# gear-genomics/tracy

Hardware: AMD Instinct MI355X
Metric: GCUPS (tracy align: Gotoh affine-gap DP cells per second, whole job) (higher is better)
Workload: dtype int16 (score sweeps) / int32 (tracebacks)

## Files before the change

include/tracy_hip.h:

```cpp
#ifndef TRACY_HIP_H
#define TRACY_HIP_H

#include <stddef.h>
#include <stdint.h>

#ifdef __cplusplus
extern "C" {
#endif

#define TRACYHIP_OK 0
#define TRACYHIP_ERR_ARG (-1)
#define TRACYHIP_ERR_HIP (-2)
#define TRACYHIP_ERR_OOM (-3)
#define TRACYHIP_ERR_RANGE (-4)
#define TRACYHIP_ERR_NODEVICE (-5)

#define TRACYHIP_MEM_HOST 0
#define TRACYHIP_MEM_DEVICE 1

#define TRACYHIP_SEQ_CHAR 0
#define TRACYHIP_SEQ_PROFILE 1

typedef struct tracyhip_ctx tracyhip_ctx;

typedef struct {
  int32_t match;
  int32_t mismatch;
  int32_t go;
  int32_t ge;
  int32_t hfree;
  int32_t vfree;
} tracyhip_params;

typedef struct {
  int32_t kind;
  const void* data;
  const uint64_t* offset;
  const uint32_t* length;
  uint32_t count;
} tracyhip_seqset;

typedef struct {
  uint32_t npairs;
  tracyhip_seqset a1;
  tracyhip_seqset a2;
  const uint32_t* a1_index;
  const uint32_t* a2_index;
} tracyhip_pairs;

int tracyhip_device_count(int* count);
int tracyhip_create(int device, tracyhip_ctx** ctx);
int tracyhip_destroy(tracyhip_ctx* ctx);
int tracyhip_set_stream(tracyhip_ctx* ctx, void* hip_stream);
int tracyhip_set_workspace_limit(tracyhip_ctx* ctx, uint64_t bytes);
int tracyhip_set_lanes(tracyhip_ctx* ctx, uint32_t lanes);
int tracyhip_synchronize(tracyhip_ctx* ctx);
int tracyhip_set_option(tracyhip_ctx* ctx, const char* name, const char* value);
int tracyhip_describe(tracyhip_ctx* ctx, char* buf, size_t cap);
int tracyhip_tune_host_allocator(void);
typedef struct {
  uint32_t traces;
  uint32_t stream_ordered;
  uint32_t host_syncs;
  uint32_t fallback_traces;
  uint32_t pruned;
  uint32_t pruned_uncertified;
  uint32_t prelim_banded;
  uint32_t prelim_repeated;
  uint32_t final_banded;
  uint32_t final_repeated;
  uint32_t allele_pruned[2];
  uint32_t allele_uncertified[2];
  uint32_t allele_banded[3];
  uint32_t allele_repeated[3];
  uint32_t allele_shared_prefix;
  uint32_t cons_fixup_columns;
  uint32_t cons_chunks;
  uint32_t asm_chunks;
  uint32_t asm_steps;
  uint32_t denovo_chunks;
  uint32_t denovo_rounds;
  uint32_t denovo_steps;
  uint32_t var_traces;
  uint32_t var_realigned;
  uint32_t var_truncated;
  uint32_t var_chunks;
  uint32_t sweep_diag_launches;
  uint32_t prefix_diag_launches;
  uint32_t band_list_pairs[2][4];
  uint32_t band_large_launches;
} tracyhip_call_stats;
int tracyhip_last_call_stats(tracyhip_ctx* ctx, tracyhip_call_stats* out);
const char* tracyhip_last_error(void);
const char* tracyhip_version(void);

int tracyhip_gotoh_score(tracyhip_ctx* ctx, const tracyhip_pairs* pairs, const tracyhip_params* prm,
                         int mem, int32_t* scores);
int tracyhip_gotoh_align(tracyhip_ctx* ctx, const tracyhip_pairs* pairs, const tracyhip_params* prm,
                         int mem, int32_t* scores, uint8_t* ops, const uint64_t* ops_offset,
                         uint32_t* ops_len);
int tracyhip_gotoh_banded(tracyhip_ctx* ctx, const tracyhip_pairs* pairs, const tracyhip_params* prm, const int32_t* band_lo,
                          const int32_t* band_hi, int mem, int32_t* scores, uint8_t* ops, const uint64_t* ops_offset, uint32_t* ops_len,
                          uint32_t* ends);
int tracyhip_needle_score(tracyhip_ctx* ctx, const tracyhip_pairs* pairs, const tracyhip_params* prm,
                          int mem, int32_t* scores);
int tracyhip_needle_align(tracyhip_ctx* ctx, const tracyhip_pairs* pairs, const tracyhip_params* prm,
                          int mem, int32_t* scores, uint8_t* ops, const uint64_t* ops_offset,
                          uint32_t* ops_len);
int tracyhip_alignment_rows(tracyhip_ctx* ctx, const tracyhip_pairs* pairs, int mem, const uint8_t* ops,
                            const uint64_t* ops_offset, const uint32_t* ops_len, uint8_t* rows0,
                            uint8_t* rows1);

typedef struct {
  uint32_t ntraces;
  tracyhip_seqset profiles;
  tracyhip_seqset refs;
  const uint32_t* ref_index;
  uint32_t trim_left;
  uint32_t trim_right;
  const uint8_t* oriented;
  uint32_t strand_by_certificate;
} tracyhip_align_job;

typedef struct {
  int32_t* score_fwd;
  int32_t* score_rev;
  uint8_t* forward;
  int32_t* score_prelim;
  uint32_t* slice_begin;
  uint32_t* slice_len;
  uint32_t* ref_pos;
  int32_t* score_final;
  uint8_t* ops;
  const uint64_t* ops_offset;
  uint32_t* ops_len;
} tracyhip_align_result;

int tracyhip_align_traces(tracyhip_ctx* ctx, const tracyhip_align_job* job, const tracyhip_params* prm,
                          int mem, const tracyhip_align_result* out);

typedef struct {
  int32_t indelshift;
  int32_t traceleft;
  uint32_t breakpoint;
  float best_diff;
} tracyhip_breakpoint;

typedef struct {
  uint32_t ntraces;
  const int32_t* signal;
  const uint64_t* signal_offset;
  const uint32_t* nsamples;
  const int32_t* bcpos;
  uint8_t* primary;
  uint8_t* secondary;
  const uint64_t* bc_offset;
  const uint32_t* bc_len;
  const int32_t* peaks;
} tracyhip_basecalls;

typedef struct {
  int32_t trim_left;
  int32_t trim_right;
  int32_t maxindel;
  int32_t madc;
} tracyhip_decomp_params;

typedef struct {
  int32_t kind;
  int32_t best_ins;
  int32_t best_del;
  int32_t best_fr;
  uint32_t dcp_n;
// ... 327 lines not shown
```

tracy_amd/capi.py:

```python
import ctypes as C
import os

import numpy as np

_HERE = os.path.dirname(os.path.abspath(__file__))

OK, ERR_ARG, ERR_HIP, ERR_OOM, ERR_RANGE, ERR_NODEVICE = 0, -1, -2, -3, -4, -5
MEM_HOST, MEM_DEVICE = 0, 1
SEQ_CHAR, SEQ_PROFILE = 0, 1


class TracyHipError(RuntimeError):
    def __init__(self, code, msg):
        super().__init__("tracyhip error %d: %s" % (code, msg))
        self.code = code


class Params(C.Structure):
    _fields_ = [("match", C.c_int32), ("mismatch", C.c_int32), ("go", C.c_int32), ("ge", C.c_int32),
                ("hfree", C.c_int32), ("vfree", C.c_int32)]


class SeqSet(C.Structure):
    _fields_ = [("kind", C.c_int32), ("data", C.c_void_p), ("offset", C.POINTER(C.c_uint64)),
                ("length", C.POINTER(C.c_uint32)), ("count", C.c_uint32)]


class Pairs(C.Structure):
    _fields_ = [("npairs", C.c_uint32), ("a1", SeqSet), ("a2", SeqSet), ("a1_index", C.POINTER(C.c_uint32)),
                ("a2_index", C.POINTER(C.c_uint32))]


class AlignJob(C.Structure):
    _fields_ = [("ntraces", C.c_uint32), ("profiles", SeqSet), ("refs", SeqSet), ("ref_index", C.POINTER(C.c_uint32)),
                ("trim_left", C.c_uint32), ("trim_right", C.c_uint32), ("oriented", C.POINTER(C.c_uint8)),
                ("strand_by_certificate", C.c_uint32)]


class AlignResult(C.Structure):
    _fields_ = [("score_fwd", C.c_void_p), ("score_rev", C.c_void_p), ("forward", C.c_void_p),
                ("score_prelim", C.c_void_p), ("slice_begin", C.c_void_p), ("slice_len", C.c_void_p),
                ("ref_pos", C.c_void_p), ("score_final", C.c_void_p), ("ops", C.c_void_p),
                ("ops_offset", C.POINTER(C.c_uint64)), ("ops_len", C.c_void_p)]


class CallStats(C.Structure):
    _fields_ = [("traces", C.c_uint32), ("stream_ordered", C.c_uint32), ("host_syncs", C.c_uint32), ("fallback_traces", C.c_uint32),
                ("pruned", C.c_uint32), ("pruned_uncertified", C.c_uint32), ("prelim_banded", C.c_uint32), ("prelim_repeated", C.c_uint32),
                ("final_banded", C.c_uint32), ("final_repeated", C.c_uint32), ("allele_pruned", C.c_uint32 * 2),
                ("allele_uncertified", C.c_uint32 * 2), ("allele_banded", C.c_uint32 * 3), ("allele_repeated", C.c_uint32 * 3),
                ("allele_shared_prefix", C.c_uint32), ("cons_fixup_columns", C.c_uint32), ("cons_chunks", C.c_uint32),
                ("asm_chunks", C.c_uint32), ("asm_steps", C.c_uint32),
                ("denovo_chunks", C.c_uint32), ("denovo_rounds", C.c_uint32), ("denovo_steps", C.c_uint32)]


class CallStatsVariants(CallStats):
    _fields_ = [("var_traces", C.c_uint32), ("var_realigned", C.c_uint32), ("var_truncated", C.c_uint32), ("var_chunks", C.c_uint32)]


class CallStatsSweeps(CallStatsVariants):
    _fields_ = [("sweep_diag_launches", C.c_uint32), ("prefix_diag_launches", C.c_uint32)]


class CallStatsBands(CallStatsSweeps):
    _fields_ = [("band_list_pairs", (C.c_uint32 * 4) * 2), ("band_large_launches", C.c_uint32)]


def library_path():
    return os.path.join(_HERE, "lib", "libtracy_hip.so")


_LIB = None


def lib():
    global _LIB
    if _LIB is None:
        p = library_path()
        if not os.path.exists(p):
            raise ImportError("tracy_amd: %s is missing -- run `python tracy_amd/build.py` (hipcc, gfx950). "
                              "There is no CPU fallback." % p)
        _LIB = C.CDLL(p)
        _LIB.tracyhip_last_error.restype = C.c_char_p
        _LIB.tracyhip_version.restype = C.c_char_p
        _LIB.tracyhip_group_context.restype = C.c_void_p
    return _LIB


def _check(rc):
    if rc != OK:
        raise TracyHipError(rc, lib().tracyhip_last_error().decode())


def device_count():
    n = C.c_int(0)
    rc = lib().tracyhip_device_count(C.byref(n))
    return n.value if rc == OK else 0


class PackedSeqs:

    def __init__(self, seqs, kind=None):
        if kind is None:
            kind = SEQ_CHAR if (len(seqs) == 0 or isinstance(seqs[0], (bytes, bytearray))) else SEQ_PROFILE
        self.kind = kind
        self.count = len(seqs)
        self.length = np.zeros(max(self.count, 1), dtype=np.uint32)
        self.offset = np.zeros(max(self.count, 1), dtype=np.uint64)
        pos = 0
        parts = []
        for i, s in enumerate(seqs):
            if kind == SEQ_CHAR:
                a = np.frombuffer(bytes(s), dtype=np.uint8)
                ln = a.size
            else:
                a = np.ascontiguousarray(s, dtype=np.float32)
                assert a.ndim == 2 and a.shape[0] == 6
                ln = a.shape[1]
                a = a.reshape(-1)
            self.length[i] = ln
            self.offset[i] = pos
            pos += a.size
            parts.append(a)
        dt = np.uint8 if kind == SEQ_CHAR else np.float32
        self.data = np.concatenate(parts) if parts and pos else np.zeros(1, dtype=dt)
        self.nelem = pos

    def seqset(self, data_ptr=None):
        s = SeqSet()
        s.kind = self.kind
        s.data = data_ptr if data_ptr is not None else self.data.ctypes.data
        s.offset = self.offset.ctypes.data_as(C.POINTER(C.c_uint64))
        s.length = self.length.ctypes.data_as(C.POINTER(C.c_uint32))
        s.count = self.count
        return s


class Context:
    def __init__(self, device=0):
        self._h = C.c_void_p()
        _check(lib().tracyhip_create(int(device), C.byref(self._h)))

    def close(self):
        if self._h:
            lib().tracyhip_destroy(self._h)
            self._h = C.c_void_p()

    def __del__(self):
        try:
            self.close()
        except Exception:
            pass

    def set_stream(self, stream_ptr):
        _check(lib().tracyhip_set_stream(self._h, C.c_void_p(stream_ptr)))

    def set_workspace_limit(self, nbytes):
        _check(lib().tracyhip_set_workspace_limit(self._h, C.c_uint64(nbytes)))

    def set_lanes(self, n):
        _check(lib().tracyhip_set_lanes(self._h, C.c_uint32(n)))

    def synchronize(self):
        _check(lib().tracyhip_synchronize(self._h))

    def set_option(self, name, value):
        _check(lib().tracyhip_set_option(self._h, str(name).encode(), str(int(value) if isinstance(value, bool) else value).encode()))

    def describe(self):
        n = lib().tracyhip_describe(self._h, None, C.c_size_t(0))
        buf = C.create_string_buffer(n)
        lib().tracyhip_describe(self._h, buf, C.c_size_t(n))
        return dict(line.split("=", 1) for line in buf.value.decode().splitlines())

    def last_call_stats(self):
        st = CallStatsBands()
        _check(lib().tracyhip_last_call_stats(self._h, C.byref(st)))
        out = {}
        for name, ty in CallStats._fields_ + CallStatsVariants._fields_ + CallStatsSweeps._fields_ + CallStatsBands._fields_:
            v = getattr(st, name)
            if name == "band_list_pairs":
                out[name] = [list(row) for row in v]
                continue
            out[name] = list(v) if hasattr(v, "__len__") else int(v)
        return out

    @staticmethod
    def _pairs(a1, a2, idx1=None, idx2=None):
        p1 = a1 if isinstance(a1, PackedSeqs) else PackedSeqs(a1)
        p2 = a2 if isinstance(a2, PackedSeqs) else PackedSeqs(a2)
        pr = Pairs()
        keep = [p1, p2]
        if idx1 is not None:
            idx1 = np.ascontiguousarray(idx1, dtype=np.uint32)
            idx2 = np.ascontiguousarray(idx2, dtype=np.uint32)
            pr.npairs = len(idx1)
            pr.a1_index = idx1.ctypes.data_as(C.POINTER(C.c_uint32))
            pr.a2_index = idx2.ctypes.data_as(C.POINTER(C.c_uint32))
            keep += [idx1, idx2]
        else:
            assert p1.count == p2.count
            pr.npairs = p1.count
        pr.a1 = p1.seqset()
        pr.a2 = p2.seqset()
        return pr, keep, p1, p2

    def _pair_lengths(self, pr, p1, p2, idx1, idx2):
        if idx1 is None:
            return p1.length[:pr.npairs].astype(np.uint64), p2.length[:pr.npairs].astype(np.uint64)
        return p1.length[np.asarray(idx1)].astype(np.uint64), p2.length[np.asarray(idx2)].astype(np.uint64)

    def score(self, a1, a2, params, needle=False, idx1=None, idx2=None):
        pr, keep, p1, p2 = self._pairs(a1, a2, idx1, idx2)
        prm = Params(*params)
        out = np.zeros(max(pr.npairs, 1), dtype=np.int32)
        fn = lib().tracyhip_needle_score if needle else lib().tracyhip_gotoh_score
        _check(fn(self._h, C.byref(pr), C.byref(prm), MEM_HOST, out.ctypes.data_as(C.POINTER(C.c_int32))))
        return out[:pr.npairs]

    def align(self, a1, a2, params, needle=False, idx1=None, idx2=None, rows=False):
        pr, keep, p1, p2 = self._pairs(a1, a2, idx1, idx2)
        prm = Params(*params)
        n = pr.npairs
        l1, l2 = self._pair_lengths(pr, p1, p2, idx1, idx2)
        cap = (l1 + l2).astype(np.uint64)
        off = np.zeros(max(n, 1), dtype=np.uint64)
        if n:
            off[1:n] = np.cumsum(cap)[:-1]
        total = int(cap.sum()) if n else 0
        ops = np.zeros(max(total, 1), dtype=np.uint8)
        olen = np.zeros(max(n, 1), dtype=np.uint32)
        scores = np.zeros(max(n, 1), dtype=np.int32)
        fn = lib().tracyhip_needle_align if needle else lib().tracyhip_gotoh_align
        _check(fn(self._h, C.byref(pr), C.byref(prm), MEM_HOST, scores.ctypes.data_as(C.POINTER(C.c_int32)),
                  ops.ctypes.data_as(C.POINTER(C.c_uint8)), off.ctypes.data_as(C.POINTER(C.c_uint64)),
                  olen.ctypes.data_as(C.POINTER(C.c_uint32))))
        btr = [ops[int(off[i]):int(off[i]) + int(olen[i])].tobytes() for i in range(n)]
        if not rows:
            return scores[:n], btr
        r0 = np.zeros(max(total, 1), dtype=np.uint8)
        r1 = np.zeros(max(total, 1), dtype=np.uint8)
        _check(lib().tracyhip_alignment_rows(self._h, C.byref(pr), MEM_HOST, ops.ctypes.data_as(C.POINTER(C.c_uint8)),
                                             off.ctypes.data_as(C.POINTER(C.c_uint64)),
                                             olen.ctypes.data_as(C.POINTER(C.c_uint32)),
                                             r0.ctypes.data_as(C.POINTER(C.c_uint8)),
                                             r1.ctypes.data_as(C.POINTER(C.c_uint8))))
        rws = [(r0[int(off[i]):int(off[i]) + int(olen[i])].tobytes(), r1[int(off[i]):int(off[i]) + int(olen[i])].tobytes())
               for i in range(n)]
        return scores[:n], btr, rws


def _align_banded(self, a1, a2, params, band_lo, band_hi, origin=False):
    pr, keep, p1, p2 = self._pairs(a1, a2, None, None)
    prm = Params(*params)
    n = pr.npairs
    l1, l2 = self._pair_lengths(pr, p1, p2, None, None)
    cap = (l1 + l2).astype(np.uint64)
    off = np.zeros(max(n, 1), dtype=np.uint64)
    if n:
        off[1:n] = np.cumsum(cap)[:-1]
    ops = np.zeros(max(int(cap.sum()) if n else 0, 1), dtype=np.uint8)
    olen = np.zeros(max(n, 1), dtype=np.uint32)
# ... 1096 lines not shown
```

tracy_amd/csrc/band16.hip:

```cpp
#include <hip/hip_runtime.h>

#include "band16.h"
#include "band16_launch.h"
#include "front.h"

namespace tracyhip {

struct DeviceWave16 {
  __device__ __forceinline__ uint32_t lane() const { return threadIdx.x; }
  __device__ __forceinline__ int32_t rot16(int32_t x) const { return __builtin_amdgcn_update_dpp(0, x, 0x121, 0xf, 0xf, false); }
  __device__ __forceinline__ int32_t rot(int32_t x, std::integral_constant<int, 16>) const { return rot16(x); }
  __device__ __forceinline__ int32_t rot(int32_t x, std::integral_constant<int, 4>) const { return __builtin_amdgcn_update_dpp(0, x, 0x93, 0xf, 0xf, false); }
  __device__ __forceinline__ uint64_t ballot(bool p) const { return __ballot(p); }
  __device__ __forceinline__ uint32_t bcast(uint32_t x, uint32_t src_lane) const { return (uint32_t)__shfl((int)x, (int)src_lane, 64); }
  __device__ __forceinline__ void sync() const { __syncthreads(); }
  __device__ __forceinline__ void sync_global() const {
    __builtin_amdgcn_fence(__ATOMIC_RELEASE, "workgroup");
    __builtin_amdgcn_fence(__ATOMIC_ACQUIRE, "workgroup");
  }
  __device__ __forceinline__ char* lds() const {
    extern __shared__ __attribute__((aligned(16))) char tracy_smem16[];
    return tracy_smem16;
  }
};

template <int K, int KIND>
__global__ __launch_bounds__(64) void band16_kernel(Band16Args a) {
  DeviceWave16 w;
  band16_body<DeviceWave16, K, KIND>(w, a, blockIdx.x);
}
template <int KIND>
__global__ __launch_bounds__(64) void band16_multi_kernel(Band16Args a12, uint32_t w12, Band16Args a8, uint32_t w8, Band16Args a4) {
  DeviceWave16 w;
  if (blockIdx.x < w12) band16_body<DeviceWave16, 12, KIND>(w, a12, blockIdx.x);
  else if (blockIdx.x < w12 + w8) band16_body<DeviceWave16, 8, KIND>(w, a8, blockIdx.x - w12);
  else band16_body<DeviceWave16, 4, KIND>(w, a4, blockIdx.x - w12 - w8);
}

template <int KIND>
__global__ __launch_bounds__(64) void band16_multi_counted_kernel(Band16Args a12, Band16Args a8, Band16Args a4, Band16Args aq) {
  DeviceWave16 w;
  const uint32_t w12 = (*a12.count + 3u) / 4u, w8 = (*a8.count + 3u) / 4u, w4 = (*a4.count + 3u) / 4u, wq = (*aq.count + 15u) / 16u;
  if (blockIdx.x < w12) band16_body<DeviceWave16, 12, KIND>(w, a12, blockIdx.x);
  else if (blockIdx.x < w12 + w8) band16_body<DeviceWave16, 8, KIND>(w, a8, blockIdx.x - w12);
  else if (blockIdx.x < w12 + w8 + w4) band16_body<DeviceWave16, 4, KIND>(w, a4, blockIdx.x - w12 - w8);
  else if (blockIdx.x < w12 + w8 + w4 + wq) band16_body<DeviceWave16, 4, KIND, false, 4>(w, aq, blockIdx.x - w12 - w8 - w4);
}

template <int KIND>
__global__ __launch_bounds__(64) void band16_multi3_counted_kernel(Band16Args a8, Band16Args a4, Band16Args aq) {
  DeviceWave16 w;
  const uint32_t w8 = (*a8.count + 3u) / 4u, w4 = (*a4.count + 3u) / 4u, wq = (*aq.count + 15u) / 16u;
  if (blockIdx.x < w8) band16_body<DeviceWave16, 8, KIND>(w, a8, blockIdx.x);
  else if (blockIdx.x < w8 + w4) band16_body<DeviceWave16, 4, KIND>(w, a4, blockIdx.x - w8);
  else if (blockIdx.x < w8 + w4 + wq) band16_body<DeviceWave16, 4, KIND, false, 4>(w, aq, blockIdx.x - w8 - w4);
}

template <int K>
__global__ __launch_bounds__(64) void band16_cont_kernel(Band16Args a) {
  DeviceWave16 w;
  band16_body<DeviceWave16, K, 1, true>(w, a, blockIdx.x);
}

template <int K>
__global__ __launch_bounds__(64) void band16_cont16_kernel(Band16Args a) {
  DeviceWave16 w;
  band16_cont16_body<DeviceWave16, K>(w, a, blockIdx.x);
}

__global__ __launch_bounds__(64) void band16_cont16_quad_kernel(Band16Args a) {
  DeviceWave16 w;
  band16_cont16_body<DeviceWave16, 4, 4>(w, a, blockIdx.x);
}

__global__ __launch_bounds__(64) void front_place_kernel(const FrontDesc* __restrict__ desc, const uint32_t* __restrict__ row, int32_t goe, int32_t halfw,
                                                         PairDesc* __restrict__ pairs, FrontOut* __restrict__ fo, const FrontOut* __restrict__ prev,
                                                         const uint32_t* __restrict__ index, const uint32_t* __restrict__ count) {
  DeviceWave16 w;
  uint32_t u = blockIdx.x;
  if (index) {
    if (u >= *count) return;
    u = index[u];
  }
  FrontDesc f = desc[u];
  if (prev && prev[u].ok) f.flags |= PAIR_SKIP;
  const FrontOut* known = (prev && !(f.flags & PAIR_SKIP) && prev[u].cstar != 0u) ? prev + u : nullptr;
  front_place_body(w, f, row, goe, halfw, pairs + u, fo + u, known);
}
__global__ __launch_bounds__(64) void front_certify_kernel(const FrontDesc* __restrict__ desc, const uint32_t* __restrict__ row, int32_t go, int32_t ge,
                                                           int32_t halfw, const int32_t* __restrict__ scores, const uint32_t* __restrict__ ends,
                                                           FrontOut* __restrict__ fo, const FrontOut* __restrict__ prev,
                                                           const uint32_t* __restrict__ index, const uint32_t* __restrict__ count) {
  DeviceWave16 w;
  uint32_t u = blockIdx.x;
  if (index) {
    if (u >= *count) return;
    u = index[u];
  }
  const FrontDesc f = desc[u];
  if (prev && prev[u].ok) return;
  front_certify_body(w, f, row, go, ge, halfw, scores[f.out], ends[2 * f.out + 1], fo + u);
}

__global__ __launch_bounds__(256) void b16_table_kernel(const B16TableDesc* __restrict__ desc, const void* __restrict__ a1, int strings,
                                                        int32_t match, int32_t mismatch, int32_t qlimit, int shift, int16_t* __restrict__ out,
                                                        int32_t* __restrict__ err) {
  const B16TableDesc d = desc[blockIdx.x];
  bool overflow = false;
  int32_t qabs = 0;
  for (uint32_t r = threadIdx.x; r < d.stride; r += blockDim.x) {
    const bool real = r < d.m;
    int32_t q[kB16Codes] = {0, 0, 0, 0, 0, 0};
    if (real) {
      b16_table_row(a1, strings != 0, d.a1_off, d.a1_stride, r, match, mismatch, q);
      if (!strings)
        for (uint32_t b = 0; b < 5; ++b) qabs = imax(qabs, q[b] < 0 ? -q[b] : q[b]);
    }
#pragma unroll
    for (uint32_t b = 0; b < kB16Codes; ++b) {
      const int32_t v = (int32_t)((uint32_t)q[b] << shift);
      overflow |= v > 32767 || v < -32768 || q[b] > 32767 || q[b] < -32768;
      out[d.out_off + (uint64_t)b * d.stride + r] = (int16_t)v;
    }
  }
  if (overflow) flag_error(err, 1);
  if (!strings && qabs > qlimit) flag_max(err, 1, qabs);
}

hipError_t launch_b16_tables(const B16TableDesc* d_desc, uint32_t nseq, const void* a1, bool strings, int32_t match, int32_t mismatch,
                             int32_t qlimit, int shift, int16_t* out, int32_t* err, hipStream_t s) {
  if (nseq == 0) return hipSuccess;
  hipLaunchKernelGGL(b16_table_kernel, dim3(nseq), dim3(256), 0, s, d_desc, a1, strings ? 1 : 0, match, mismatch, qlimit, shift, out, err);
  return hipGetLastError();
}

hipError_t launch_band16(int K, int kind, const Band16Args& a, hipStream_t s) {
  if (a.npairs == 0) return hipSuccess;
  const dim3 grid((a.npairs + 3u) / 4u);
  const uint32_t lds = 4u * a.code_cap + b16_table_bytes(K);
#define TRACY_B16(KK)                                                                                     \
  case KK:                                                                                                \
    if (kind == 0) hipLaunchKernelGGL((band16_kernel<KK, 0>), grid, dim3(64), lds, s, a);                 \
    else hipLaunchKernelGGL((band16_kernel<KK, 1>), grid, dim3(64), lds, s, a);                           \
    break;
  switch (K) {
    TRACY_B16(4) TRACY_B16(8) TRACY_B16(12)
    default: return hipErrorInvalidValue;
  }
#undef TRACY_B16
  return hipGetLastError();
}

hipError_t launch_band16_multi(int kind, const Band16Args& a12, const Band16Args& a8, const Band16Args& a4, hipStream_t s) {
  const uint32_t w12 = (a12.npairs + 3u) / 4u, w8 = (a8.npairs + 3u) / 4u, w4 = (a4.npairs + 3u) / 4u;
  if (w12 + w8 + w4 == 0) return hipSuccess;
  const uint32_t lds = 4u * a12.code_cap + b16_table_bytes(12);
  if (kind == 0) hipLaunchKernelGGL((band16_multi_kernel<0>), dim3(w12 + w8 + w4), dim3(64), lds, s, a12, w12, a8, w8, a4);
  else hipLaunchKernelGGL((band16_multi_kernel<1>), dim3(w12 + w8 + w4), dim3(64), lds, s, a12, w12, a8, w8, a4);
  return hipGetLastError();
}

hipError_t B16Fork::create() {
  hipError_t e;
  int least = 0, greatest = 0;
  if (hipDeviceGetStreamPriorityRange(&least, &greatest) != hipSuccess) { (void)hipGetLastError(); least = greatest = 0; }
  const bool flat = getenv("TRACYHIP_NO_STREAM_PRIORITY") != nullptr;
  for (int i = 0; i < kSide; ++i) {
    const int prio = (!flat && i == 3) ? least : 0;
    (void)greatest;
    if ((e = hipStreamCreateWithPriority(&side[i], hipStreamNonBlocking, prio)) != hipSuccess) return e;
// ... 3 lines not shown
    if ((e = hipEventCreateWithFlags(&r, hipEventDisableTiming)) != hipSuccess) return e;
  return hipEventCreateWithFlags(&forked, hipEventDisableTiming);
}
void B16Fork::destroy() {
  for (int i = 0; i < kSide; ++i) {
    if (side[i]) (void)hipStreamDestroy(side[i]);
    if (joined[i]) (void)hipEventDestroy(joined[i]);
    side[i] = nullptr; joined[i] = nullptr;
  }
  for (auto& r : ready) { if (r) (void)hipEventDestroy(r); r = nullptr; }
  if (forked) (void)hipEventDestroy(forked);
  forked = nullptr;
}

hipError_t launch_band16_counted(int kind, const Band16Args& a12, const Band16Args& a8, const Band16Args& a4, const Band16Args& aq, hipStream_t s,
                                 const B16Fork* fork, uint32_t multi_max, bool* large) {
  if (large) *large = false;
  uint32_t most = a12.npairs;
  for (uint32_t x : {a8.npairs, a4.npairs, aq.npairs}) most = x > most ? x : most;
  if (most == 0) return hipSuccess;
  hipError_t e;
  if (most <= multi_max) {
    const uint32_t lds16 = 4u * a12.code_cap + b16_table_bytes(12), ldsq = aq.npairs ? b16_quad_lds(aq.code_cap) : 0u;
    const uint32_t lds = lds16 > ldsq ? lds16 : ldsq;
    const dim3 grid((most + 3u) / 4u + 4u);
    if (kind == 0) hipLaunchKernelGGL((band16_multi_counted_kernel<0>), grid, dim3(64), lds, s, a12, a8, a4, aq);
    else hipLaunchKernelGGL((band16_multi_counted_kernel<1>), grid, dim3(64), lds, s, a12, a8, a4, aq);
    return hipGetLastError();
  }
  if (large) *large = true;
  const uint32_t lds16 = 4u * a8.code_cap + b16_table_bytes(8), ldsq = aq.npairs ? b16_quad_lds(aq.code_cap) : 0u;
  const uint32_t lds = lds16 > ldsq ? lds16 : ldsq;
  const dim3 grid((most + 3u) / 4u + 3u);
  if (fork) {
    if ((e = hipEventRecord(fork->forked, s)) != hipSuccess) return e;
    if ((e = hipStreamWaitEvent(fork->side[2], fork->forked, 0)) != hipSuccess) return e;
  }
  if (kind == 0) hipLaunchKernelGGL((band16_multi3_counted_kernel<0>), grid, dim3(64), lds, s, a8, a4, aq);
  else hipLaunchKernelGGL((band16_multi3_counted_kernel<1>), grid, dim3(64), lds, s, a8, a4, aq);
  if ((e = hipGetLastError()) != hipSuccess) return e;
  if ((e = launch_band16(12, kind, a12, fork ? fork->side[2] : s)) != hipSuccess) return e;
  if (fork) {
    if ((e = hipEventRecord(fork->joined[2], fork->side[2])) != hipSuccess) return e;
    if ((e = hipStreamWaitEvent(s, fork->joined[2], 0)) != hipSuccess) return e;
  }
  return hipSuccess;
}

hipError_t launch_band16_cont_quad(const Band16Args& a, hipStream_t s) {
  if (a.npairs == 0) return hipSuccess;
  hipLaunchKernelGGL(band16_cont16_quad_kernel, dim3((a.npairs + 15u) / 16u), dim3(64), b16_cont_quad_lds(a.code_cap), s, a);
  return hipGetLastError();
}

hipError_t launch_band16_cont(int K, const Band16Args& a, hipStream_t s, bool narrow) {
  if (a.npairs == 0) return hipSuccess;
  const dim3 grid((a.npairs + 3u) / 4u);
  const uint32_t lds = narrow ? b16_cont16_lds(K, a.code_cap) : 4u * a.code_cap + b16_table_bytes(K) + 4u * 2u * kB16RowCap * 4u;
  if (narrow) {
    switch (K) {
      case 12: hipLaunchKernelGGL((band16_cont16_kernel<12>), grid, dim3(64), lds, s, a); break;
      case 8: hipLaunchKernelGGL((band16_cont16_kernel<8>), grid, dim3(64), lds, s, a); break;
      case 4: hipLaunchKernelGGL((band16_cont16_kernel<4>), grid, dim3(64), lds, s, a); break;
      default: return hipErrorInvalidValue;
    }
    return hipGetLastError();
  }
  switch (K) {
    case 12: hipLaunchKernelGGL((band16_cont_kernel<12>), grid, dim3(64), lds, s, a); break;
    case 8: hipLaunchKernelGGL((band16_cont_kernel<8>), grid, dim3(64), lds, s, a); break;
    case 4: hipLaunchKernelGGL((band16_cont_kernel<4>), grid, dim3(64), lds, s, a); break;
    default: return hipErrorInvalidValue;
  }
  return hipGetLastError();
}

hipError_t launch_front_place(const FrontDesc* d_desc, uint32_t n, const uint32_t* row, int32_t goe, int32_t halfw, PairDesc* d_pairs, FrontOut* d_fo,
                              hipStream_t s, const FrontOut* d_prev, const uint32_t* d_index, const uint32_t* d_count) {
  if (n == 0) return hipSuccess;
  hipLaunchKernelGGL(front_place_kernel, dim3(n), dim3(64), 0, s, d_desc, row, goe, halfw, d_pairs, d_fo, d_prev, d_index, d_count);
  return hipGetLastError();
}

hipError_t launch_front_certify(const FrontDesc* d_desc, uint32_t n, const uint32_t* row, int32_t go, int32_t ge, int32_t halfw, const int32_t* d_scores,
                                const uint32_t* d_ends, FrontOut* d_fo, hipStream_t s, const FrontOut* d_prev, const uint32_t* d_index,
                                const uint32_t* d_count) {
  if (n == 0) return hipSuccess;
  hipLaunchKernelGGL(front_certify_kernel, dim3(n), dim3(64), 0, s, d_desc, row, go, ge, halfw, d_scores, d_ends, d_fo, d_prev, d_index, d_count);
  return hipGetLastError();
}

}
```

tracy_amd/csrc/band16_launch.h:

```cpp
#ifndef TRACY_AMD_BAND16_LAUNCH_H
#define TRACY_AMD_BAND16_LAUNCH_H

#include <hip/hip_runtime.h>

#include "band16.h"

namespace tracyhip {

struct B16TableDesc {
  uint64_t a1_off;
  uint64_t out_off;
  uint32_t a1_stride;
  uint32_t m;
  uint32_t stride;
  uint32_t pad;
};

hipError_t launch_b16_tables(const B16TableDesc* d_desc, uint32_t nseq, const void* a1, bool strings, int32_t match, int32_t mismatch,
                             int32_t qlimit, int shift, int16_t* out, int32_t* err, hipStream_t s);
hipError_t launch_band16(int K, int kind, const Band16Args& a, hipStream_t s);
hipError_t launch_band16_multi(int kind, const Band16Args& a12, const Band16Args& a8, const Band16Args& a4, hipStream_t s);
struct B16Fork {
  static constexpr int kSide = 4;
  hipStream_t side[kSide] = {nullptr, nullptr, nullptr, nullptr};
  hipEvent_t forked = nullptr, joined[kSide] = {nullptr, nullptr, nullptr, nullptr};
  hipEvent_t ready[2] = {nullptr, nullptr};
  hipError_t create();
  void destroy();
};
#ifndef TRACY_B16_MULTI_MAX
#define TRACY_B16_MULTI_MAX 49152u
#endif
hipError_t launch_band16_counted(int kind, const Band16Args& a12, const Band16Args& a8, const Band16Args& a4, const Band16Args& aq, hipStream_t s,
                                 const B16Fork* fork = nullptr, uint32_t multi_max = TRACY_B16_MULTI_MAX, bool* large = nullptr);
hipError_t launch_band16_cont(int K, const Band16Args& a, hipStream_t s, bool narrow = false);
hipError_t launch_band16_cont_quad(const Band16Args& a, hipStream_t s);
struct FrontDesc;
struct FrontOut;
hipError_t launch_front_place(const FrontDesc* d_desc, uint32_t n, const uint32_t* row, int32_t goe, int32_t halfw, PairDesc* d_pairs, FrontOut* d_fo,
                              hipStream_t s, const FrontOut* d_prev = nullptr, const uint32_t* d_index = nullptr, const uint32_t* d_count = nullptr);
hipError_t launch_front_certify(const FrontDesc* d_desc, uint32_t n, const uint32_t* row, int32_t go, int32_t ge, int32_t halfw, const int32_t* d_scores,
                                const uint32_t* d_ends, FrontOut* d_fo, hipStream_t s, const FrontOut* d_prev = nullptr, const uint32_t* d_index = nullptr,
                                const uint32_t* d_count = nullptr);

}
#endif
```

tracy_amd/csrc/capi.hip:

```cpp
#include <hip/hip_runtime.h>
#include <atomic>
#include <sched.h>
#include <malloc.h>
#include <map>
#include <chrono>

#include <thread>

#include <algorithm>
#include <cctype>
#include <cstdarg>
#include <cstddef>
#include <cstdio>
#include <cstdlib>
#include <cstring>
#include <string>
#include <memory>
#include <vector>

#include "../../include/tracy_hip.h"
#include "capi_internal.h"
#include "launch.h"
#include "stream_plan.h"
#include "sweep_range.h"
// ... 128 lines not shown
      {
        std::unique_lock<std::mutex> lk(m);
        cv.wait(lk, [&] { return gen != seen; });
        seen = gen;
        j = job;
      }
      slices(*j);
      {
        std::lock_guard<std::mutex> lk(m);
        if (--pending == 0) done_cv.notify_one();
      }
    }
  }
  static uint32_t share() {
    uint32_t want = kHostThreads;
    if (const char* e = getenv("TRACYHIP_HOST_THREADS")) { const int v = atoi(e); if (v >= 1) want = (uint32_t)v; }
    else {
      cpu_set_t set;
      CPU_ZERO(&set);
      if (sched_getaffinity(0, sizeof(set), &set) == 0) { const int c = CPU_COUNT(&set); if (c >= 1) want = (uint32_t)c; }
      if (FILE* f = fopen("/sys/fs/cgroup/cpu.max", "r")) {
        char quota[32] = {0};
        unsigned long period = 0;
        if (fscanf(f, "%31s %lu", quota, &period) == 2 && period > 0 && strcmp(quota, "max") != 0) {
          const unsigned long q = strtoul(quota, nullptr, 10) / period;
          if (q >= 1 && q < want) want = (uint32_t)q;
        }
        fclose(f);
      }
    }
    return want > kHostThreads ? kHostThreads : want;
  }
  bool run(const std::function<void(uint32_t)>& f) {
    std::unique_lock<std::mutex> u(use, std::try_to_lock);
    if (!u.owns_lock()) return false;
    if (!started) {
      const uint32_t want = share();
      nworkers = want - 1;
      for (uint32_t t = 0; t < nworkers; ++t) std::thread([this] { worker(); }).detach();
      started = true;
    }
    {
      std::lock_guard<std::mutex> lk(m);
      job = &f;
      next.store(0);
      pending = nworkers;
      ++gen;
    }
    if (nworkers) cv.notify_all();
    slices(f);
    std::unique_lock<std::mutex> lk(m);
    done_cv.wait(lk, [&] { return pending == 0; });
    return true;
  }
};
}
uint32_t host_pool_threads() {
  static const uint32_t n = HostPool::share();
  return n;
}
bool host_pool_run(const std::function<void(uint32_t)>& job) {
  static HostPool* pool = new HostPool;
  return pool->run(job);
}

HostScope::HostScope(const char* l) : label(l), t0(host_profile().on ? now_ns() : 0) {}
HostScope::~HostScope() {
  HostProfile& p = host_profile();
  if (!p.on) return;
  const double ms = (double)(now_ns() - t0) * 1e-6;
  std::lock_guard<std::mutex> lk(p.m);
  auto& e = p.acc[label];
  e.first += ms;
  e.second += 1;
}

namespace {
struct KnobField { const char* name; bool CtxKnobs::*flag; };
const KnobField kKnobFlags[] = {
    {"no_stream", &CtxKnobs::no_stream}, {"no_narrow", &CtxKnobs::no_narrow}, {"no_compact", &CtxKnobs::no_compact},
    {"no_screen", &CtxKnobs::no_screen}, {"no_band", &CtxKnobs::no_band}, {"no_band16", &CtxKnobs::no_band16},
    {"no_front", &CtxKnobs::no_front}, {"no_prefix", &CtxKnobs::no_prefix}, {"no_vote", &CtxKnobs::no_vote},
    {"no_origin", &CtxKnobs::no_origin}, {"no_subwindow", &CtxKnobs::no_subwindow}, {"no_prelim_origin", &CtxKnobs::no_prelim_origin},
    {"no_cq", &CtxKnobs::no_cq}, {"no_fused_walk", &CtxKnobs::no_fused_walk}, {"no_cont16", &CtxKnobs::no_cont16}, {"no_decomp_wave", &CtxKnobs::no_decomp_wave}, {"no_af_split", &CtxKnobs::no_af_split}, {"no_front_lists", &CtxKnobs::no_front_lists}, {"no_origin_band", &CtxKnobs::no_origin_band}, {"no_quads", &CtxKnobs::no_quads}, {"no_fork", &CtxKnobs::no_fork}, {"no_early_tail", &CtxKnobs::no_early_tail}, {"sweeps_alone", &CtxKnobs::sweeps_alone}, {"no_sweep_diag", &CtxKnobs::no_sweep_diag}, {"verbose", &CtxKnobs::verbose}};
bool same_name(const char* a, const char* b) {
  for (; *a && *b; ++a, ++b)
    if (std::tolower((unsigned char)*a) != std::tolower((unsigned char)*b)) return false;
  return *a == *b;
}
}
bool knobs_set(CtxKnobs& k, const char* name, const char* value) {
  if (!name || !value) return false;
  if (same_name(name, "band_w")) {
    char* end = nullptr;
    const long v = strtol(value, &end, 10);
    if (end == value) return false;
    k.band_w = v < 0 ? -1 : (int32_t)std::min<long>(4096, v);
    return true;
  }
  if (same_name(name, "quad_tier_min")) {
    const long v = atol(value);
    if (v < 0) return false;
    k.quad_tier_min = (uint32_t)std::min<long>(v, 0x7fffffffl);
    return true;
  }
  if (same_name(name, "front_list_min")) {
    const long v = atol(value);
    if (v < 0) return false;
    k.front_list_min = (uint32_t)std::min<long>(v, 0x7fffffffl);
    return true;
  }
  if (same_name(name, "b16_multi_max")) {
    char* end = nullptr;
    const long v = strtol(value, &end, 10);
    if (end == value || *end || v < 0 || v > 0x7fffffffl) return false;
    k.b16_multi_max = (uint32_t)v;
    return true;
  }
  if (same_name(name, "seed_vote_cap")) {
    const long v = atol(value);
    if (v < 1 || v > 2048) return false;
    k.seed_vote_cap = (uint32_t)v;
    return true;
  }
  if (same_name(name, "sweep_diag_period")) {
    const long v = atol(value);
    if (v != 0 && (v < 64 || v > 32768 || v % 4 != 0)) return false;
    k.sweep_diag_period = (uint32_t)v;
    return true;
  }
  if (same_name(name, "ckpt_b")) {
    const long v = atol(value);
    if (v < 32 || v > 1024) return false;
    k.ckpt_b = (uint32_t)v;
    return true;
  }
  for (const KnobField& f : kKnobFlags)
    if (same_name(name, f.name)) {
      k.*(f.flag) = !(value[0] == '0' && value[1] == 0);
      return true;
    }
  return false;
}
void knobs_from_env(CtxKnobs& k) {
  for (const KnobField& f : kKnobFlags) {
    std::string env = "TRACYHIP_";
    for (const char* c = f.name; *c; ++c) env.push_back((char)std::toupper((unsigned char)*c));
    if (getenv(env.c_str())) k.*(f.flag) = true;
  }
  if (getenv("TRACYHIP_HOST_TIMERS")) k.verbose = true;
  if (const char* e = getenv("TRACYHIP_BAND_W")) knobs_set(k, "band_w", e);
  if (const char* e = getenv("TRACYHIP_CKPT_B")) knobs_set(k, "ckpt_b", e);
  if (const char* e = getenv("TRACYHIP_QUAD_TIER_MIN")) knobs_set(k, "quad_tier_min", e);
  if (const char* e = getenv("TRACYHIP_FRONT_LIST_MIN")) knobs_set(k, "front_list_min", e);
  if (const char* e = getenv("TRACYHIP_B16_MULTI_MAX")) knobs_set(k, "b16_multi_max", e);
  if (const char* e = getenv("TRACYHIP_SEED_VOTE_CAP")) knobs_set(k, "seed_vote_cap", e);
  if (const char* e = getenv("TRACYHIP_SWEEP_DIAG_PERIOD")) knobs_set(k, "sweep_diag_period", e);
}
std::string knobs_describe(const CtxKnobs& k) {
  std::string s;
  for (const KnobField& f : kKnobFlags) { s += f.name; s += k.*(f.flag) ? "=1\n" : "=0\n"; }
  s += "band_w=" + std::to_string(k.band_w) + "\n";
  s += "ckpt_b=" + std::to_string(k.ckpt_b) + "\n";
  s += "quad_tier_min=" + std::to_string(k.quad_tier_min) + "\n";
  s += "front_list_min=" + std::to_string(k.front_list_min) + "\n";
  s += "b16_multi_max=" + std::to_string(k.b16_multi_max) + "\n";
  s += "seed_vote_cap=" + std::to_string(k.seed_vote_cap) + "\n";
// ... 1422 lines not shown
```

tracy_amd/csrc/capi_internal.h:

```cpp
#ifndef TRACY_AMD_CAPI_INTERNAL_H
#define TRACY_AMD_CAPI_INTERNAL_H

#include <hip/hip_runtime.h>

#include <atomic>
#include <condition_variable>
#include <deque>
#include <functional>
#include <mutex>
#include <string>
#include <thread>
#include <utility>
#include <vector>

#include "../../include/tracy_hip.h"
#include "assemble_wave.h"
#include "dp_kernels.h"
#include "band16_launch.h"
#include "front.h"

namespace tracyhip {

struct DevBuf {
  void* p = nullptr;
// ... 91 lines not shown
  AB_OFF,
  AB_LEN,
  AB_W0,
  AB_W1,
  AB_SPAN,
  AB_PROF,
  AB_PCLASS,
  AB_STEP,
  AB_PAY,
  DN_PROF = AB_TR,
  DN_SEQS = AB_SEQS,
  DN_CLASS = AB_CLASS,
  DN_COLCLASS = AB_PCLASS,
  DN_TABLE = AB_SC2,
  DN_OPS = AB_OPS,
  DN_OFF = AB_OFF,
  DN_LEN = AB_LEN,
  DN_ROWS = AB_W0,
  DN_SPAN = AB_SPAN,
  DN_STEP = AB_STEP,
  DN_PAY = AB_PAY,
  DN_CNT,
  VB_DESC,
  VB_EVENTS,
  VB_LEN,
  VB_PAIRS,
  VB_RCDESC,
  VB_SEQ,
  VB_OPS,
  VB_OPS_OFF,
  VB_OPS_LEN,
  VB_IN_PRIMARY,
  VB_IN_SECDECOMP,
  VB_IN_REFS,
  VB_IN_OPS0,
  VB_IN_OPS1,
  VB_OUT_REC,
  VB_OUT_TEXT,
  VB_OUT_N,
  VB_PACK_OFF,
  VB_PACK_REC,
  VB_PACK_TEXT,
  DB_COUNT
};
static_assert(DN_CNT + 1 == VB_DESC && VB_PACK_TEXT + 1 == DB_COUNT && DN_PAY < DB_COUNT,
              "an alias does not advance the count: every slot of its own comes after the aliases");
enum CtxPin : int {
  PB_DESC,
  PB_OFF,
  PB_TMP,
  PB_RES,
  PB_PRE,
  PB_B16DESC0,
  PB_COUNT = PB_B16DESC0 + 4
};

int set_error(int code, const char* fmt, ...);
#define HIP_TRY(expr)                                                                               \
  do {                                                                                              \
    hipError_t _e = (expr);                                                                         \
    if (_e != hipSuccess)                                                                           \
      return set_error(_e == hipErrorOutOfMemory ? TRACYHIP_ERR_OOM : TRACYHIP_ERR_HIP, "%s failed: %s (%s:%d)", \
                       #expr, hipGetErrorString(_e), __FILE__, __LINE__);                           \
  } while (0)

struct CtxKnobs {
  bool no_stream = false;
  bool no_narrow = false;
  bool no_compact = false;
  bool no_screen = false;
  bool no_band = false;
  bool no_band16 = false;
  bool no_front = false;
  bool no_prefix = false;
  bool no_vote = false;
  bool no_origin = false;
  bool no_subwindow = false;
  bool no_prelim_origin = false;
  bool no_cq = false;
  bool no_fused_walk = false;
  bool no_quads = false;
  bool no_fork = false;
  bool no_early_tail = false;
  bool sweeps_alone = false;
  bool no_sweep_diag = false;
  bool no_origin_band = false;
  bool no_front_lists = false;
  bool no_af_split = false;
  bool no_decomp_wave = false;
  bool no_cont16 = false;
  bool verbose = false;
  int32_t band_w = -1;
  uint32_t ckpt_b = 256;
  uint32_t sweep_diag_period = 0;
  uint32_t b16_multi_max = TRACY_B16_MULTI_MAX;
  uint32_t front_list_min = 1024;
  uint32_t seed_vote_cap = 2048;
  uint32_t quad_tier_min = 32768;
};
void knobs_from_env(CtxKnobs& k);
bool knobs_set(CtxKnobs& k, const char* name, const char* value);
std::string knobs_describe(const CtxKnobs& k);

constexpr size_t kCodePad = 128;
int choose_k(uint32_t m, int mode, bool needle = false);
uint64_t seqset_extent(const tracyhip_seqset& s);

struct DpProblem {
  int mode = MODE_CHAR;
  bool a1_profile = false, a2_profile = false;
  const void* d_a1 = nullptr;
  const void* d_a2 = nullptr;
  const void* d_a2_chars = nullptr;
  const uint8_t* d_special = nullptr;
  int cq_codes = 6;
  const uint8_t* d_colclass = nullptr;
  std::vector<PairDesc> desc;
  std::vector<int> k;
};

}

struct tracyhip_ctx {
  int device = 0;
  hipStream_t stream = nullptr;
  hipStream_t own_stream = nullptr;
  uint64_t ws_limit = 0;
  tracyhip::DevBuf dev[tracyhip::DB_COUNT];
  tracyhip::PinBuf pin[tracyhip::PB_COUNT];
  std::vector<tracyhip::PairDesc> cache_desc;
  std::vector<int> cache_k;
  std::vector<tracyhip::PairDesc> cache_full, cache_pre, cache_b16;
  std::vector<tracyhip::FrontDesc> cache_fd;
  std::vector<int> cache_fullk, cache_b16k;
  tracyhip::B16Fork b16_fork;
  bool b16_fork_ok = false;
  bool cons_gq_ready = false;
  hipError_t ensure_codes(size_t bytes, hipStream_t st) {
    tracyhip::DevBuf &d_codes = dev[tracyhip::DB_CODES], &d_special = dev[tracyhip::DB_SPECIAL];
    hipError_t e = d_codes.ensure(bytes + 2 * tracyhip::kCodePad);
    if (e != hipSuccess) return e;
    if ((e = hipMemsetAsync(d_codes.p, 0, tracyhip::kCodePad, st)) != hipSuccess) return e;
    if ((e = hipMemsetAsync(static_cast<uint8_t*>(d_codes.p) + tracyhip::kCodePad + bytes, 0, tracyhip::kCodePad, st)) != hipSuccess) return e;
    if ((e = d_special.ensure((bytes >> 8) + 2)) != hipSuccess) return e;
    return hipMemsetAsync(d_special.p, 0, (bytes >> 8) + 2, st);
  }
  uint8_t* special_blocks() const { return static_cast<uint8_t*>(dev[tracyhip::DB_SPECIAL].p); }
  uint8_t* codes() const { return static_cast<uint8_t*>(dev[tracyhip::DB_CODES].p) + tracyhip::kCodePad; }
  bool aftab_ready = false;
  uint64_t ws_cache_budget = 0, ws_cache_held = 0;
  uint32_t ws_cache_share = 0;
  bool declut_ready = false;
  uint32_t b16_round = 0;
  struct Pending { int which; hipEvent_t e0, e1; uint64_t cells, bytes; };
  std::vector<tracyhip_ctx*> lanes;
  uint32_t mem_share = 1;
  bool timing = false;
  tracyhip::CtxKnobs knobs;
  tracyhip_call_stats stats = {};
  std::vector<Pending> pending;
  std::vector<hipEvent_t> free_events;
  tracyhip_kernel_timing acc[TRACYHIP_TIMER_COUNT] = {};
  struct AsyncState {
    std::mutex m;
    std::condition_variable cv;
    std::deque<std::function<int()>> q;
// ... 167 lines not shown
```

tracy_amd/csrc/dp_kernels.h:

```cpp
#ifndef TRACY_AMD_DP_KERNELS_H
#define TRACY_AMD_DP_KERNELS_H

#include "dp_lane.h"

#if defined(__HIP_DEVICE_COMPILE__)
#define TRACY_KEEP_BRANCH() asm volatile("" ::: "memory")
#else
#define TRACY_KEEP_BRANCH() ((void)0)
#endif

namespace tracyhip {

enum : int { MODE_CHAR = 0, MODE_QP = 1, MODE_PROF = 2, MODE_CQ = 3 };
TR_HD constexpr bool qp_like(int mode) { return mode == MODE_QP || mode == MODE_CQ; }
TR_HD uint32_t cq_code(uint8_t c) { return c == 'A' ? 0u : c == 'C' ? 1u : c == 'G' ? 2u : c == 'T' ? 3u : c == 'N' ? 4u : 5u; }
TR_HD bool cq_row_char(uint8_t c) { return c == 'A' || c == 'C' || c == 'G' || c == 'T' || c == 'N'; }
enum : uint32_t {
  PAIR_A2_REVCOMP = 1u,
  PAIR_ROW4_ZERO = 2u,
  PAIR_BANDED = 4u,
  PAIR_KEEP_ROW = 8u,
  PAIR_SKIP = 16u,
};

// ... 502 lines not shown
#pragma unroll
          for (int k = 0; k < 5; ++k) nb[k] = a2p[(uint64_t)k * d.a2_stride + ci];
        }
        bool screen_on = screen_pair;
        uint32_t nfail = 0;
        const uint8_t* cls = screen_on ? a.colcode + d.a2_off : nullptr;
        uint32_t ncls = kColClassOther;
        if (screen_on) {
          sub.screen_setup();
          ncls = cls[col_at(1 - (int32_t)L)];
        }
        for (uint32_t t = 1; t <= t_end; ++t) {
#pragma unroll
          for (int k = 0; k < 5; ++k) sub.b[k] = nb[k];
          const uint32_t ccls = ncls;
          const uint32_t ci = col_at((int32_t)t - (int32_t)L + 1);
#pragma unroll
          for (int k = 0; k < 5; ++k) nb[k] = a2p[(uint64_t)k * d.a2_stride + ci];
          if (screen_on) {
            ncls = cls[ci];
            int32_t bad = sub.screen();
            if (ccls < kColClassOther) {
              const int16_t* tp = qp_tab + qp6_index<K>(ccls, 0u, L);
#pragma unroll
              for (int i = 0; i < K; ++i) sub.sv[i] = (int32_t)((uint32_t)(int32_t)tp[i * 64] << SH);
              bad = 0;
            }
            if (w.ballot(bad < 0) != 0) {
              sub.prepare();
              if (++nfail > 64u && 2u * nfail > t) screen_on = false;
            }
          } else {
            sub.prepare();
          }
          do_step(t, sub);
        }
      };
      auto sweep4 = [&]() {
        SubProf<K, 4> s4;
#pragma unroll
        for (int i = 0; i < K; ++i)
#pragma unroll
          for (int k = 0; k < 5; ++k) s4.a[i][k] = sub_p.a[i][k];
        s4.fmatch = fmatch; s4.fmis = fmis; s4.shift = SH;
        sweep(s4);
      };
      if constexpr (NT == 4) sweep4();
      else if constexpr (NT == 5) sweep(sub_p);
      else { if (skip4) sweep4(); else sweep(sub_p); }
    }
    (void)T;

    if (BOTTOM) {
      if (a.scores && L == lanes_used - 1) a.scores[d.out] = NARROW ? sext16(bot_h - goe) : bot_h;
    } else if (last_pass && a.scores) {
      const uint32_t g = m - 1 - base;
      if (L == g / K) {
        int32_t v = 0;
#pragma unroll
        for (int i = 0; i < K; ++i)
          if ((uint32_t)i == g % K) v = TRACE ? (ts.Hc[i] >> SH) : ((NARROW || A16) ? sext16(ss.Hl[i]) : ss.Hl[i]);
        a.scores[d.out] = v;
      }
    }
    if (!last_pass) w.sync_global();
  }
}

template <bool G>
struct SweepGuard { static constexpr bool value = G; };

template <int K>
struct QpStrip {
  uint32_t v[K];
  TR_HD int32_t lo16(int i) const { return (int32_t)v[i]; }
};
TR_HD constexpr uint32_t lds_bytes_sweep16(int K, bool compact) { return (compact ? 4u : 6u) * 256u * (uint32_t)((K + 1) / 2); }
TR_HD constexpr uint32_t lds_bytes_prefix(int K, bool compact) { return lds_bytes_sweep16(K, compact); }
template <int NC>
TR_HD constexpr uint32_t qp16_row_byte(uint32_t row) { return (row >> 1) * ((uint32_t)NC * 256u) + (row & 1u) * 128u; }
template <int NC>
TR_HD uint32_t qp16_byte(uint32_t code, uint32_t row, uint32_t lanecol) { return qp16_row_byte<NC>(row) + code * 256u + 2u * lanecol; }
template <class W>
TR_HD bool reference_is_plain(W& w, const DpArgs& a, const PairDesc& d) {
  if (!a.special_blocks) return false;
  if (d.n == 0) return true;
  const uint64_t first = d.a2_off >> 8, last = (d.a2_off + d.n - 1) >> 8;
  uint32_t seen = 0;
  for (uint64_t b = first + w.lane(); b <= last; b += 64) seen |= a.special_blocks[b];
  return w.ballot(seen != 0) == 0;
}
template <int K, int NC>
TR_HD void qp_fetch6(const char* tab, uint32_t addr, QpStrip<K>& q) {
#if defined(__HIP_DEVICE_COMPILE__)
#pragma unroll
  for (int i = 0; i < K; ++i) asm volatile("ds_read_u16 %0, %1 offset:%2" : "=v"(q.v[i]) : "v"(addr), "n"(qp16_row_byte<NC>((uint32_t)i)));
#else
  for (int i = 0; i < K; ++i) {
    uint16_t x;
    __builtin_memcpy(&x, tab + addr + qp16_row_byte<NC>((uint32_t)i), 2);
    q.v[i] = x;
  }
#endif
}
template <int K>
TR_HD void qp_wait6(QpStrip<K>& q) {
#if defined(__HIP_DEVICE_COMPILE__)
  constexpr int newer = K < 15 ? K : 15;
#define TR_TIE4(o) "+v"(q.v[o]), "+v"(q.v[o + 1]), "+v"(q.v[o + 2]), "+v"(q.v[o + 3])
  if constexpr (K == 15) asm volatile("s_waitcnt lgkmcnt(%15)" : TR_TIE4(0), TR_TIE4(4), TR_TIE4(8), "+v"(q.v[12]), "+v"(q.v[13]), "+v"(q.v[14]) : "n"(newer));
  else if constexpr (K == 16) asm volatile("s_waitcnt lgkmcnt(%16)" : TR_TIE4(0), TR_TIE4(4), TR_TIE4(8), TR_TIE4(12) : "n"(newer));
  else if constexpr (K == 12) asm volatile("s_waitcnt lgkmcnt(%12)" : TR_TIE4(0), TR_TIE4(4), TR_TIE4(8) : "n"(newer));
  else if constexpr (K == 8) asm volatile("s_waitcnt lgkmcnt(%8)" : TR_TIE4(0), TR_TIE4(4) : "n"(newer));
  else if constexpr (K == 4) asm volatile("s_waitcnt lgkmcnt(%4)" : TR_TIE4(0) : "n"(newer));
  else asm volatile("s_waitcnt lgkmcnt(0)" ::: "memory");
#undef TR_TIE4
#endif
}

TR_HD int32_t lastrow_h(const int32_t* lr, uint32_t c, bool narrow) { return narrow ? sext16(lr[c]) : lr[2 * c]; }
TR_HD int32_t lastrow_e(const int32_t* lr, uint32_t c, bool narrow, int32_t goe) { return narrow ? (lr[c] >> 16) + goe : lr[2 * c + 1]; }

template <class W, int K, bool CKPT, bool COMPACT, bool STRINGS, bool DIAG>
TR_HD void gotoh_narrow_qp_body(W& w, const DpArgs& a, uint32_t pair_idx) {
  const PairDesc d = a.pairs[pair_idx];
  if (d.flags & PAIR_SKIP) return;
  if (reference_is_plain(w, a, d) != COMPACT) return;
  const uint32_t L = w.lane();
  const uint32_t m = d.m, n = d.n;
  const int32_t go = a.go, ge = a.ge, goe = go + ge;
  if (m == 0 || n == 0) {
    if (L == 0 && a.scores) a.scores[d.out] = (m == 0) ? 0 : edge_value(false, go, ge, (int32_t)m);
    return;
  }
  const float* a1p = static_cast<const float*>(a.a1) + (STRINGS ? 0 : d.a1_off);
  const uint8_t* a1c = static_cast<const uint8_t*>(a.a1) + (STRINGS ? d.a1_off : 0);
  const uint8_t* a2c = static_cast<const uint8_t*>(a.a2) + d.a2_off;
  constexpr int NC = COMPACT ? 4 : 6;
  int16_t* qp_tab = reinterpret_cast<int16_t*>(w.lds());
  const float fmatch = (float)a.match, fmis = (float)a.mismatch;
  const uint32_t lanes_used = (m + K - 1) / K;
  const uint32_t pad = lanes_used * K - m;
  const uint32_t t_end = n + lanes_used - 1;
  const bool rcflag = (d.flags & PAIR_A2_REVCOMP) != 0;
  const bool lastlane = L == lanes_used - 1;

  int32_t Hl[K], El[K];
#pragma unroll
  for (int i = 0; i < K; ++i) {
    const uint32_t r = L * K + i + 1 - pad;
    if constexpr (DIAG) {
      const int32_t rr = (int32_t)(L * K + i + 1) - (int32_t)pad;
      if (rr <= 0) { Hl[i] = rr * -ge; El[i] = -goe + (rr - 1) * -ge; }
      else { Hl[i] = go; El[i] = kNegInf16 + (rr - 1) * -ge; }
    } else if (L * K + i < pad) { Hl[i] = 0; El[i] = -goe; }
    else { Hl[i] = edge_value(false, go, ge, (int32_t)r); El[i] = kNegInf16; }
  }
  int32_t gev = ge, goev = DIAG ? go : goe;
  int32_t hext_last = lastlane ? (DIAG ? -ge : 0) : (DIAG ? 0 : ge);
  int32_t delta_last = lastlane ? -goe : 0;
#if defined(__HIP_DEVICE_COMPILE__)
  asm volatile("" : "+v"(gev), "+v"(goev), "+v"(hext_last), "+v"(delta_last));
#endif

  const uint32_t Lc = ((L & 31u) << 1) | (L >> 5);
  {
    bool overflow = false;
    int32_t qabs = 0;
#pragma unroll 1
    for (int i = 0; i < K; ++i) {
      const uint32_t r = L * K + i + 1 - pad;
      const bool real = r - 1 < m;
      float pr[5] = {0.0f, 0.0f, 0.0f, 0.0f, 0.0f};
// ... 1217 lines not shown
```

tracy_amd/csrc/dp_kernels.hip:

```cpp
#include <hip/hip_runtime.h>

#include <cstdlib>

#include "dp_kernels.h"
#include "launch.h"

namespace tracyhip {

static uint32_t lds_pad() {
  static int v = -1;
  if (v < 0) { const char* e = getenv("TRACYHIP_LDS_PAD"); v = e ? atoi(e) : 0; }
  return (uint32_t)v;
}

struct DeviceWave {
  __device__ __forceinline__ uint32_t lane() const { return threadIdx.x; }
  __device__ __forceinline__ int32_t shift_up(int32_t x) const {
    return __builtin_amdgcn_update_dpp(0, x, 0x138, 0xf, 0xf, true);
  }
  __device__ __forceinline__ int32_t shift_up_row(int32_t x) const {
    return __builtin_amdgcn_update_dpp(0, x, 0x111, 0xf, 0xf, true);
  }
  __device__ __forceinline__ int32_t shift_up_or(int32_t x, int32_t first) const {
    return __builtin_amdgcn_update_dpp(first, x, 0x138, 0xf, 0xf, false);
// ... 424 lines not shown
  if (mode == MODE_CHAR) return launch_band_m<MODE_CHAR>(K, a, wa, npairs, s);
  if (mode == MODE_QP) return launch_band_m<MODE_QP>(K, a, wa, npairs, s);
  return hipErrorInvalidValue;
}

hipError_t launch_gotoh_origin(int K, int table, int codes, const DpArgs& a, uint32_t npairs, hipStream_t s) {
  if (npairs == 0) return hipSuccess;
  if (table == 2) {
#define TRACY_ORIGIN_QP(KK)                                                                                                            \
  case KK:                                                                                                                              \
    if (a.special_blocks) hipLaunchKernelGGL((gotoh_origin_kernel<KK, 2, 4>), dim3(npairs), dim3(64), 4u * 64u * KK * 2u + lds_pad(), s, a); \
    hipLaunchKernelGGL((gotoh_origin_kernel<KK, 2, 6>), dim3(npairs), dim3(64), lds_bytes(MODE_QP, KK), s, a);                              \
    break;
    switch (K) {
      TRACY_ORIGIN_QP(4) TRACY_ORIGIN_QP(8) TRACY_ORIGIN_QP(12) TRACY_ORIGIN_QP(15) TRACY_ORIGIN_QP(16)
      default: return hipErrorInvalidValue;
    }
#undef TRACY_ORIGIN_QP
    return hipGetLastError();
  }
  if (table) {
#define TRACY_ORIGIN_CASE(KK)                                                                                                          \
  case KK:                                                                                                                              \
    if (codes <= 4) hipLaunchKernelGGL((gotoh_origin_kernel<KK, 1, 4>), dim3(npairs), dim3(64), 4u * 64u * KK * 2u + lds_pad(), s, a);      \
    else if (codes == 5) hipLaunchKernelGGL((gotoh_origin_kernel<KK, 1, 5>), dim3(npairs), dim3(64), 5u * 64u * KK * 2u + lds_pad(), s, a); \
    else hipLaunchKernelGGL((gotoh_origin_kernel<KK, 1, 6>), dim3(npairs), dim3(64), lds_bytes(MODE_CQ, KK), s, a);                          \
    break;
    switch (K) {
      TRACY_ORIGIN_CASE(4) TRACY_ORIGIN_CASE(8) TRACY_ORIGIN_CASE(12) TRACY_ORIGIN_CASE(15) TRACY_ORIGIN_CASE(16)
      default: return hipErrorInvalidValue;
    }
#undef TRACY_ORIGIN_CASE
    return hipGetLastError();
  }
  switch (K) {
    case 4: hipLaunchKernelGGL((gotoh_origin_kernel<4>), dim3(npairs), dim3(64), 0, s, a); break;
    case 8: hipLaunchKernelGGL((gotoh_origin_kernel<8>), dim3(npairs), dim3(64), 0, s, a); break;
    case 12: hipLaunchKernelGGL((gotoh_origin_kernel<12>), dim3(npairs), dim3(64), 0, s, a); break;
    case 15: hipLaunchKernelGGL((gotoh_origin_kernel<15>), dim3(npairs), dim3(64), 0, s, a); break;
    case 16: hipLaunchKernelGGL((gotoh_origin_kernel<16>), dim3(npairs), dim3(64), 0, s, a); break;
    default: return hipErrorInvalidValue;
  }
  return hipGetLastError();
}

static constexpr uint32_t lds_combo(int K, bool compact) {
  const uint32_t pre = lds_bytes_prefix(K, compact), sw = lds_bytes_sweep16(K, compact);
  return pre > sw ? pre : sw;
}
hipError_t launch_gotoh_ckpt_prefix(int K, const DpArgs& full, uint32_t nfull, const DpArgs& pre, uint32_t npre, hipStream_t s) {
  if (nfull + npre == 0) return hipSuccess;
  constexpr int GL = kPrefixLanes;
  const dim3 grid(nfull + (npre + 64 / GL - 1) / (64 / GL));
#define TRACY_COMBO_CASE(KK)                                                                                            \
  case KK:                                                                                                              \
    if constexpr (KK == 15 || KK == 16) {                                                                               \
      if (combo_uses_diag<KK>(full, nfull, pre, npre)) {                                                                \
        if (full.special_blocks)                                                                                        \
          hipLaunchKernelGGL((gotoh_ckpt_prefix_kernel<KK, GL, true, KK, true>), grid, dim3(64), lds_combo(KK, true), s, full, nfull, pre, npre); \
        hipLaunchKernelGGL((gotoh_ckpt_prefix_kernel<KK, GL, false, KK, true>), grid, dim3(64), lds_combo(KK, false), s, full, nfull, pre, npre); \
        break;                                                                                                          \
      }                                                                                                                 \
    }                                                                                                                   \
    if (full.special_blocks) {                                                                                          \
      hipLaunchKernelGGL((gotoh_ckpt_prefix_kernel<KK, GL, true>), grid, dim3(64), lds_combo(KK, true), s, full, nfull, pre, npre); \
      hipLaunchKernelGGL((gotoh_ckpt_prefix_kernel<KK, GL, false>), grid, dim3(64), lds_combo(KK, false), s, full, nfull, pre, npre); \
    } else {                                                                                                            \
      hipLaunchKernelGGL((gotoh_ckpt_prefix_kernel<KK, GL, false>), grid, dim3(64), lds_combo(KK, false), s, full, nfull, pre, npre); \
    }                                                                                                                   \
    break;
  switch (K) {
    TRACY_COMBO_CASE(4) TRACY_COMBO_CASE(8) TRACY_COMBO_CASE(12) TRACY_COMBO_CASE(15) TRACY_COMBO_CASE(16)
    default: return hipErrorInvalidValue;
  }
#undef TRACY_COMBO_CASE
  return hipGetLastError();
}

static uint32_t front_prefix_tall_min() {
  static const uint32_t v = [] { const char* e = getenv("TRACYHIP_PREFIX_TALL_MIN"); return e ? (uint32_t)strtoul(e, nullptr, 10) : 40000u; }();
  return v;
}
template <int GL, int KP>
static hipError_t launch_gotoh_ckpt_front_t(int K, const DpArgs& full, uint32_t nfull, const DpArgs& pre, uint32_t npre, hipStream_t s) {
  static_assert(GL * KP == (int)kFrontRows, "the rows above the kept one");
  const dim3 grid(nfull + (npre + 64 / GL - 1) / (64 / GL));
  auto lds = [](int KK, bool compact) {
    const uint32_t pre_b = lds_bytes_prefix(KP, compact), sw = lds_bytes_sweep16(KK, compact);
    return (pre_b > sw ? pre_b : sw) + lds_pad();
  };
#define TRACY_FRONT_CASE(KK)                                                                                            \
  case KK:                                                                                                              \
    if constexpr (KK == 15 || KK == 16) {                                                                               \
      if (combo_uses_diag<KK>(full, nfull, pre, npre)) {                                                                \
        if (full.special_blocks)                                                                                        \
          hipLaunchKernelGGL((gotoh_ckpt_prefix_kernel<KK, GL, true, KP, true>), grid, dim3(64), lds(KK, true), s, full, nfull, pre, npre); \
        hipLaunchKernelGGL((gotoh_ckpt_prefix_kernel<KK, GL, false, KP, true>), grid, dim3(64), lds(KK, false), s, full, nfull, pre, npre); \
        break;                                                                                                          \
      }                                                                                                                 \
    }                                                                                                                   \
    if (full.special_blocks) {                                                                                          \
       \
       \
      hipLaunchKernelGGL((gotoh_ckpt_prefix_kernel<KK, GL, true, KP>), grid, dim3(64), lds(KK, true), s, full, nfull, pre, npre); \
      hipLaunchKernelGGL((gotoh_ckpt_prefix_kernel<KK, GL, false, KP>), grid, dim3(64), lds(KK, false), s, full, nfull, pre, npre); \
    } else {                                                                                                            \
      hipLaunchKernelGGL((gotoh_ckpt_prefix_kernel<KK, GL, false, KP>), grid, dim3(64), lds(KK, false), s, full, nfull, pre, npre); \
    }                                                                                                                   \
    break;
  switch (K) {
    TRACY_FRONT_CASE(4) TRACY_FRONT_CASE(8) TRACY_FRONT_CASE(12) TRACY_FRONT_CASE(15) TRACY_FRONT_CASE(16)
    default: return hipErrorInvalidValue;
  }
#undef TRACY_FRONT_CASE
  return hipGetLastError();
}
hipError_t launch_gotoh_ckpt_front(int K, const DpArgs& full, uint32_t nfull, const DpArgs& pre, uint32_t npre, hipStream_t s) {
  if (nfull + npre == 0) return hipSuccess;
  if (nfull == 0 && npre >= front_prefix_tall_min()) return launch_gotoh_ckpt_front_t<(int)kFrontRows / 16, 16>(K, full, nfull, pre, npre, s);
  return launch_gotoh_ckpt_front_t<kFrontPrefixLanes, kFrontPrefixK>(K, full, nfull, pre, npre, s);
}

hipError_t launch_gotoh_prefix(int K, const DpArgs& a, uint32_t npairs, hipStream_t s) {
  if (npairs == 0) return hipSuccess;
  constexpr int GL = kPrefixLanes;
  const dim3 grid((npairs + 64 / GL - 1) / (64 / GL));
#define TRACY_PREFIX_CASE(KK) \
  case KK:                                                                                                                      \
    hipLaunchKernelGGL((gotoh_prefix_kernel<KK, GL, false>), grid, dim3(64), lds_bytes_prefix(KK, false), s, a, npairs);                        \
    if (a.special_blocks) hipLaunchKernelGGL((gotoh_prefix_kernel<KK, GL, true>), grid, dim3(64), lds_bytes_prefix(KK, true), s, a, npairs); \
    break;
  switch (K) {
    TRACY_PREFIX_CASE(4) TRACY_PREFIX_CASE(8) TRACY_PREFIX_CASE(12) TRACY_PREFIX_CASE(15) TRACY_PREFIX_CASE(16)
    default: return hipErrorInvalidValue;
  }
#undef TRACY_PREFIX_CASE
  return hipGetLastError();
}
template <int GL, int KP>
static hipError_t launch_gotoh_front_prefix_cq_t(const DpArgs& a, uint32_t npairs, hipStream_t s) {
  const dim3 grid((npairs + 64 / GL - 1) / (64 / GL));
  hipLaunchKernelGGL((gotoh_prefix_kernel<KP, GL, false, true>), grid, dim3(64), lds_bytes_prefix(KP, false), s, a, npairs);
  if (a.special_blocks) hipLaunchKernelGGL((gotoh_prefix_kernel<KP, GL, true, true>), grid, dim3(64), lds_bytes_prefix(KP, true), s, a, npairs);
  return hipGetLastError();
}
hipError_t launch_gotoh_front_prefix_cq(const DpArgs& a, uint32_t npairs, hipStream_t s) {
  if (npairs == 0) return hipSuccess;
  if (npairs >= front_prefix_tall_min()) return launch_gotoh_front_prefix_cq_t<(int)kFrontRows / 16, 16>(a, npairs, s);
  return launch_gotoh_front_prefix_cq_t<kFrontPrefixLanes, kFrontPrefixK>(a, npairs, s);
}
hipError_t launch_gotoh_walk(const WalkArgs& a, hipStream_t s) {
  if (a.npairs == 0) return hipSuccess;
  hipLaunchKernelGGL(gotoh_walk_kernel, dim3(a.npairs), dim3(64), 0, s, a);
  return hipGetLastError();
}
hipError_t launch_needle_walk(const WalkArgs& a, const uint32_t* bits32, hipStream_t s) {
  if (a.npairs == 0) return hipSuccess;
  hipLaunchKernelGGL(needle_walk_kernel, dim3((a.npairs + 63) / 64), dim3(64), 0, s, a, bits32);
  return hipGetLastError();
}
hipError_t launch_alignment_rows(const RowsArgs& a, hipStream_t s) {
  if (a.npairs == 0) return hipSuccess;
  hipLaunchKernelGGL(alignment_rows_kernel, dim3(a.npairs), dim3(64), 0, s, a);
  return hipGetLastError();
}

}
```

tracy_amd/csrc/front.h:

```cpp
#ifndef TRACY_AMD_FRONT_H
#define TRACY_AMD_FRONT_H

#include "band16.h"

namespace tracyhip {

constexpr int kFrontK = 12;
constexpr int32_t kFrontHalfW = 90;

struct FrontDesc {
  uint64_t row_off;
  uint64_t a2_off;
  uint64_t tab_off;
  uint32_t tab_stride;
  uint32_t m_rest;
  uint32_t n;
  uint32_t flags;
  uint32_t out;
  uint32_t R;
  int32_t rest;
  uint32_t tight;
};
struct FrontOut {
  int32_t vmax;
  uint32_t cstar;
  uint32_t shift;
  uint32_t ok;
};

TR_HD int32_t front_v(uint32_t x, int32_t goe) {
  const int32_t h = sext16((int32_t)x) - goe, f = (int32_t)x >> 16;
  return h > f ? h : f;
}

template <class W>
TR_HD void front_place_body(W& w, const FrontDesc& f, const uint32_t* row, int32_t goe, int32_t halfw, PairDesc* pair, FrontOut* fo,
                            const FrontOut* known = nullptr) {
  const uint32_t L = w.lane();
  if (f.flags & PAIR_SKIP) {
    if (L == 0) {
      PairDesc d{};
      d.flags = PAIR_SKIP;
      d.out = f.out;
      *pair = d;
      *fo = FrontOut{0, 0u, 0u, 0u};
    }
    return;
  }
  int32_t vmax = INT32_MIN;
  uint32_t cstar = 0;
  if (known) {
    vmax = known->vmax;
    cstar = known->cstar;
  } else {
    const uint32_t* r = row + f.row_off;
    int32_t best = INT32_MIN;
    uint32_t bc = 0;
    constexpr uint32_t kRounds = 8;
    for (uint32_t c0 = 1u; c0 <= f.n; c0 += 64u * kRounds) {
      uint32_t x[kRounds];
#pragma unroll
      for (uint32_t u = 0; u < kRounds; ++u) {
        const uint32_t c = c0 + 64u * u + L;
        x[u] = r[c <= f.n ? c : f.n];
      }
#pragma unroll
      for (uint32_t u = 0; u < kRounds; ++u) {
        const uint32_t c = c0 + 64u * u + L;
        const int32_t v = front_v(x[u], goe);
        const bool take = c <= f.n && v > best;
        best = take ? v : best;
        bc = take ? c : bc;
      }
    }
    for (uint32_t l = 0; l < 64u; ++l) {
      const int32_t v = (int32_t)w.bcast((uint32_t)best, l);
      const uint32_t c = w.bcast(bc, l);
      if (c != 0 && (v > vmax || (v == vmax && c < cstar))) { vmax = v; cstar = c; }
    }
  }
  if (L != 0) return;
  const int32_t dlo = (int32_t)cstar - halfw, dhi = (int32_t)cstar + halfw;
  const uint32_t a = dlo > 1 ? (uint32_t)(dlo - 1) : 0u;
  uint32_t nsub = f.n - a;
  const uint64_t reach = (uint64_t)f.m_rest + (uint64_t)(dhi - (int32_t)a) + 1ull;
  if ((uint64_t)nsub > reach) nsub = (uint32_t)reach;
  PairDesc d{};
  d.a1_off = f.tab_off;
  d.a1_stride = f.tab_stride;
  d.m = f.m_rest;
  d.n = nsub;
  d.a2_stride = nsub;
  d.a2_off = (f.flags & PAIR_A2_REVCOMP) ? f.a2_off + (uint64_t)(f.n - a - nsub) : f.a2_off + a;
  d.out = f.out;
  d.flags = f.flags & PAIR_A2_REVCOMP;
  d.ckpt_off = band_pack(dlo - (int32_t)a, dhi - (int32_t)a);
  d.lastrow_off = f.row_off + a;
  d.bits_off = f.R;
  *pair = d;
  fo->vmax = vmax;
  fo->cstar = cstar;
  fo->shift = a;
  fo->ok = 0;
}

template <class W>
TR_HD void front_certify_body(W& w, const FrontDesc& f, const uint32_t* row, int32_t go, int32_t ge, int32_t halfw, int32_t score, uint32_t c_end,
                              FrontOut* fo) {
  const uint32_t L = w.lane();
  if (f.flags & PAIR_SKIP) return;
  const uint32_t* r = row + f.row_off;
  const int32_t goe = go + ge;
  const int64_t age = -(int64_t)ge;
  const int64_t dlo = (int64_t)fo->cstar - halfw, dhi = (int64_t)fo->cstar + halfw;
  const bool two = f.tight != 0u && age >= 2;
  const int64_t rest1 = (int64_t)f.rest - ((int64_t)f.tight - 1);
  const int64_t q = age - 1;
  bool bad = false, bad1 = false;
  constexpr uint32_t kRounds = 8;
  for (uint32_t c0 = 0; c0 <= f.n; c0 += 64u * kRounds) {
    uint32_t x[kRounds];
#pragma unroll
    for (uint32_t u = 0; u < kRounds; ++u) {
      const uint32_t c = c0 + 64u * u + L;
      x[u] = f.n ? r[c == 0 ? 1u : c <= f.n ? c : f.n] : 0u;
    }
#pragma unroll
    for (uint32_t u = 0; u < kRounds; ++u) {
      const uint32_t c = c0 + 64u * u + L;
      const int64_t v = c == 0 ? (int64_t)edge_value(false, go, ge, (int32_t)f.R) : (int64_t)front_v(x[u], goe);
      const int64_t cc = (int64_t)c;
      const bool live = c <= f.n;
      const bool inside = cc >= dlo && cc <= dhi;
      const int64_t margin = inside ? (cc - dlo < dhi - cc ? cc - dlo : dhi - cc) : -1;
      bad = bad || (live && v + (int64_t)f.rest - age * (margin + 1) >= (int64_t)score);
      if (two) {
        const int64_t ph = age * (dhi - cc + 1), pv = q * (cc - dlo + 1);
        const int64_t pen = inside ? (ph < pv ? ph : pv) : 0;
        bad1 = bad1 || (live && v + rest1 - pen >= (int64_t)score);
      }
    }
  }
  const bool any = w.ballot(bad) != 0;
  const bool any1 = !two || w.ballot(bad1) != 0;
  if (L == 0) fo->ok = ((!any || !any1) && c_end != 0) ? 1u : 0u;
}

}
#endif
```

tracy_amd/csrc/launch.h:

```cpp
#ifndef TRACY_AMD_LAUNCH_H
#define TRACY_AMD_LAUNCH_H

#include <hip/hip_runtime.h>

#include "dp_kernels.h"

namespace tracyhip {

struct RowsArgs {
  const PairDesc* pairs;
  const void* a1;
  const void* a2;
  int32_t a1_profile, a2_profile;
  int32_t a2_revcomp_flag;
  int32_t a2_onehot;
  const uint8_t* ops;
  const uint64_t* ops_off;
  const uint32_t* ops_len;
  uint8_t* rows0;
  uint8_t* rows1;
  uint32_t npairs;
  const int32_t* row0_gaps_only;
  uint32_t row0_gaps_only_stride;
};

hipError_t launch_gotoh(int mode, int K, bool trace, bool narrow, const DpArgs& a, uint32_t npairs, hipStream_t s, bool rawtab = false);
hipError_t launch_gotoh_front_prefix_cq(const DpArgs& a, uint32_t npairs, hipStream_t s);
hipError_t launch_gotoh_prof(int K, bool trace, bool row4_zero, bool arith16, const DpArgs& a, uint32_t npairs, hipStream_t s);
hipError_t launch_gotoh_ckpt(int mode, int K, bool narrow, const DpArgs& a, uint32_t npairs, hipStream_t s);
hipError_t launch_band_trace(int mode, int K, const DpArgs& a, const WalkArgs& wa, uint32_t npairs, hipStream_t s);
hipError_t launch_gotoh_origin(int K, int table, int codes, const DpArgs& a, uint32_t npairs, hipStream_t s);
hipError_t launch_gotoh_ckpt_prefix(int K, const DpArgs& full, uint32_t nfull, const DpArgs& pre, uint32_t npre, hipStream_t s);
hipError_t launch_gotoh_prefix(int K, const DpArgs& a, uint32_t npairs, hipStream_t s);
hipError_t launch_gotoh_ckpt_front(int K, const DpArgs& full, uint32_t nfull, const DpArgs& pre, uint32_t npre, hipStream_t s);
hipError_t launch_needle(int mode, int K, bool trace, const DpArgs& a, uint32_t npairs, hipStream_t s);
hipError_t launch_gotoh_walk(const WalkArgs& a, hipStream_t s);
hipError_t launch_needle_walk(const WalkArgs& a, const uint32_t* bits32, hipStream_t s);
hipError_t launch_alignment_rows(const RowsArgs& a, hipStream_t s);

}
#endif
```

tracy_amd/csrc/stream.hip:

```cpp
#include <hip/hip_runtime.h>

#include <algorithm>
#include <cstring>
#include <numeric>
#include <string>
#include <type_traits>
#include <vector>

#include "../../include/tracy_hip.h"
#include "capi_internal.h"
#include "decompose_launch.h"
#include "launch.h"
#include "pipe_internal.h"
#include "pipe_kernels.h"
#include "stream_fields.h"
#include "stream_plan.h"

using namespace tracyhip;

#define TRY(expr) do { const int _rc = (expr); if (_rc) return _rc; } while (0)

namespace {

struct Arena {
// ... 59 lines not shown
  const uint32_t R = kFrontRows;
  const SOrient o = s_orient_class(votes[2 * t], votes[2 * t + 1], G.mt, (G.flags & SG_FRONT_OK) != 0u, p.exact != 0u);
  const uint32_t g = o.g, cls = o.cls;
  PairDesc fa = s_skip_pair(t), fb = s_skip_pair(t), pa = s_skip_pair(t), pb = s_skip_pair(t);
  FrontDesc f{};
  f.flags = PAIR_SKIP;
  f.out = t;
  uint64_t cells = 0, bytes = 0, pcells = 0;
  const uint64_t full_cells = (uint64_t)G.mt * G.rn, pre_cells = (uint64_t)(G.mt < R ? G.mt : R) * G.rn, full_bytes = 24ull * G.mt + G.rn + 4;
  if (cls == 0u) {
    pa = s_stage1_desc(G, t, p.nt, g);
    pa.flags |= PAIR_KEEP_ROW;
    pcells += pre_cells;
    if (p.exact) { fa = s_stage1_desc(G, t, p.nt, 1u - g); cells += full_cells; bytes += full_bytes; }
    else { pb = s_stage1_desc(G, t, p.nt, 1u - g); pcells += pre_cells; }
    f.row_off = G.lr_off[g];
    f.a2_off = G.ref_off;
    f.tab_off = G.tab_off + G.tl + R;
    f.tab_stride = G.tab_stride;
    f.m_rest = G.mt - R;
    f.n = G.rn;
    f.flags = g ? PAIR_A2_REVCOMP : 0u;
    f.R = R;
    f.rest = ub[t];
    f.tight = (p.ge <= -2 && ub1[t] <= ub[t]) ? (uint32_t)(ub[t] - ub1[t]) + 1u : 0u;
    s_count(lc, SC_FRONT_CELLS, s_front_cells(f.m_rest));
    s_count(lc, SC_FRONT_BYTES, s_front_bytes(f.m_rest, f.n));
  } else if (cls == 1u) {
    fa = s_stage1_desc(G, t, p.nt, g);
    fb = s_stage1_desc(G, t, p.nt, 1u - g);
    cells += 2 * full_cells; bytes += 2 * full_bytes;
  } else {
    fa = s_stage1_desc(G, t, p.nt, g);
    pb = s_stage1_desc(G, t, p.nt, 1u - g);
    cells += full_cells; pcells += pre_cells; bytes += full_bytes;
  }
  if (p.split_prefix) { s_count(lc, SC_FRONT_CELLS, pcells); s_count(lc, SC_FRONT_BYTES, pcells ? (uint64_t)R + 5ull * G.rn : 0ull); }
  else cells += pcells;
  full[G.full_a] = fa;
  full[G.full_b] = fb;
  pre[t] = pa;
  if (!p.exact) pre[p.nt + t] = pb;
  fd[t] = f;
  STrace S{};
  S.g = (uint8_t)g;
  S.cls = (uint8_t)cls;
  tr[t] = S;
  s_count(lc, SC_SWEEP_CELLS, cells);
  s_count(lc, SC_SWEEP_BYTES, bytes);
  });
}

__device__ __forceinline__ uint32_t s_front_result(uint32_t t, const FrontOut* __restrict__ fo1, const int32_t* __restrict__ fs1, const uint32_t* __restrict__ fe1,
                                                   const FrontOut* __restrict__ fo2, const int32_t* __restrict__ fs2, const uint32_t* __restrict__ fe2, int64_t* s_g) {
  if (fo1[t].ok) { *s_g = fs1[t]; return fe1[2 * t + 1] ? fe1[2 * t + 1] + fo1[t].shift : 0u; }
  if (fo2[t].ok) { *s_g = fs2[t]; return fe2[2 * t + 1] ? fe2[2 * t + 1] + fo2[t].shift : 0u; }
  return 0u;
}

__global__ void s_orient_early_kernel(SParams p, const FrontOut* __restrict__ fo1,
                                      const int32_t* __restrict__ fs1, const uint32_t* __restrict__ fe1, const FrontOut* __restrict__ fo2,
                                      const int32_t* __restrict__ fs2, const uint32_t* __restrict__ fe2, STrace* __restrict__ tr) {
  const uint32_t t = blockIdx.x * blockDim.x + threadIdx.x;
  if (t >= p.nt) return;
  STrace S = tr[t];
  if (S.cls != 0u || !p.use_votes || !p.exact) return;
  const uint32_t g = S.g;
  int64_t s_g = 0;
  const uint32_t fce = s_front_result(t, fo1, fs1, fe1, fo2, fs2, fe2, &s_g);
  if (fce == 0u) return;
  S.sc[g] = (int32_t)s_g;
  S.fwd = g == 0u ? 1 : 0;
  S.rc = (uint8_t)g;
  S.sstar = (int32_t)s_g;
  S.ce = fce;
  S.mark = ST_EARLY;
  tr[t] = S;
}

__global__ void s_orient_decide_kernel(SParams p, const SGeom* __restrict__ geom, const uint32_t* __restrict__ votes, const int32_t* __restrict__ ub,
                                       const int32_t* __restrict__ sc2, const FrontOut* __restrict__ fo1, const int32_t* __restrict__ fs1,
                                       const uint32_t* __restrict__ fe1, const FrontOut* __restrict__ fo2, const int32_t* __restrict__ fs2,
                                       const uint32_t* __restrict__ fe2, STrace* __restrict__ tr, RowEndDesc* __restrict__ re,
                                       uint32_t* __restrict__ dead, unsigned long long* __restrict__ cnt, PairDesc* __restrict__ desc_trim) {
  with_counters(cnt, [&](unsigned long long* lc) {
  const uint32_t t = blockIdx.x * blockDim.x + threadIdx.x;
  if (t >= p.nt) return;
  const SGeom G = geom[t];
  STrace S = tr[t];
  const uint32_t g = S.g, o = 1u - g, nt = p.nt;
  uint32_t dd = 0;
  int64_t s_g = 0, s_o = 0;
  uint32_t fce = 0;
  auto by_bound = [&]() {
    const SStrand c = s_strand_by_bound(g, sc2[o * nt + t], ub[t], s_g);
    if (c.certified) s_o = c.bound;
    else dd |= SD_STRAND;
  };
  if (S.cls == 0u) {
    s_count(lc, SC_PRUNED);
    fce = s_front_result(t, fo1, fs1, fe1, fo2, fs2, fe2, &s_g);
    if (fce == 0u) { dd |= SD_FRONT; s_count(lc, SC_PRUNED_UNCERT); }
    else if (p.exact) s_o = sc2[o * nt + t];
    else by_bound();
  } else if (S.cls == 1u) {
    s_g = sc2[g * nt + t];
    s_o = sc2[o * nt + t];
  } else {
    s_g = sc2[g * nt + t];
    by_bound();
  }
  S.sc[g] = (int32_t)s_g;
  S.sc[o] = (int32_t)s_o;
  const bool fwd = S.sc[0] > S.sc[1];
  S.fwd = fwd ? 1 : 0;
  S.rc = fwd ? 0 : 1;
  const uint32_t w = S.rc;
  S.sstar = S.sc[w];
  const bool from_front = S.cls == 0u && w == g;
  if (!dd && !from_front) {
    const bool swept = S.cls == 1u || (S.cls == 0u && p.exact) || (S.cls == 2u && w == g);
    if (!swept) dd |= SD_STRAND;
    else if (p.use_votes && vote_skips_checkpoints(votes[2 * t], votes[2 * t + 1], w)) dd |= SD_LOSER_WON;
  }
  S.ce = from_front ? fce : 0u;
  re[t] = RowEndDesc{G.lr_off[w], (from_front || dd) ? 0u : G.rn, 0u};
  tr[t] = S;
  if (dd && (S.mark & ST_EARLY)) {
    dead[t] = dd;
    if (S.mark & ST_COUNTED_PRELIM) s_count(lc, SC_PRELIM_BANDED, ~0ull);
    if (S.mark & ST_COUNTED_FINAL) s_count(lc, SC_FINAL_BANDED, ~0ull);
  } else if (dd) dead[t] |= dd;
  if (desc_trim) {
    PairDesc d{};
    d.a1_off = G.prof_off + G.tl; d.a1_stride = G.mf; d.m = G.mt;
    d.a2_off = G.ref_off; d.n = G.rn; d.a2_stride = G.rn;
    d.out = t;
    d.flags = S.rc ? PAIR_A2_REVCOMP : 0u;
    desc_trim[t] = d;
  }
  });
}

__global__ void s_prelim_plan_kernel(SParams p, int mode, int early, const SGeom* __restrict__ geom, STrace* __restrict__ tr, const uint32_t* __restrict__ d_ce,
                                     const int32_t* __restrict__ top, uint32_t* __restrict__ dead, PairDesc* __restrict__ cand,
                                     uint8_t* __restrict__ kc) {
  const uint32_t t = blockIdx.x * blockDim.x + threadIdx.x;
  if (t >= p.nt) return;
  kc[t] = 0;
  STrace S = tr[t];
  if (((S.mark & ST_EARLY) != 0u) != (early != 0)) return;
  if (dead[t]) return;
  const SGeom G = geom[t];
  const bool from_front = S.cls == 0 && S.rc == S.g;
  const uint32_t ce = from_front ? S.ce : d_ce[t];
  S.ce = ce;
  uint32_t dd = 0;
  if (ce == 0u) dd = SD_JUNK;
  else {
    const SubWindow sw = s_sub_window(G.mt, ce, top[t], S.sstar, p.ge);
    S.gap = (uint32_t)(sw.g < 0x7fffffff ? sw.g : 0x7fffffff);
    S.shift = sw.a;
    int K = sw.K;
    if (K && mode == 0 && !b16_origin_ok(p.match, p.mismatch, p.go, p.ge, G.mt, sw.n)) K = 0;
    if (K && !s_fits_lds(sw.n, K)) K = 0;
    if (!K) dd = SD_PRELIM_BAND;
    else if (sw.n > p.ncap) dd = SD_SHAPE;
    else {
      PairDesc q{};
      q.a1_off = G.tab_off + G.tl;
      q.a1_stride = G.tab_stride;
      q.m = G.mt;
      q.n = sw.n;
      q.a2_stride = sw.n;
      q.a2_off = G.ref_off + (S.rc ? (uint64_t)(G.rn - ce) : (uint64_t)sw.a);
      q.flags = S.rc ? PAIR_A2_REVCOMP : 0u;
      q.out = t;
      q.ckpt_off = band_pack(sw.dlo, sw.dhi);
      q.lastrow_off = mode == 0 ? 0ull : ((uint64_t)(G.rn - ce) | ((uint64_t)sw.a << 32));
      cand[t] = q;
      kc[t] = (uint8_t)K;
    }
  }
// ... 128 lines not shown
  s_count(lc, SC_PRELIM_BANDED);
  if (early) S.mark |= ST_COUNTED_PRELIM;
  const uint32_t m = G.mf, n = S.trim.len;
  const SFinalBand fb = s_final_band(m, n, s_final_width(S.gap));
  uint32_t dd = 0;
  if (!fb.K) dd = SD_FINAL_BAND;
  else if (n > p.ncap) dd = SD_SHAPE;
  else {
    S.bw = (int32_t)fb.w;
    PairDesc q{};
    q.a1_off = G.tab_off;
    q.a1_stride = G.tab_stride;
    q.m = m;
    q.n = n;
    q.a2_stride = n;
    q.a2_off = G.ref_off + (S.rc ? G.rn - S.trim.ri - S.trim.len : S.trim.ri);
    q.flags = S.rc ? PAIR_A2_REVCOMP : 0u;
    q.out = t;
    q.ckpt_off = band_pack(fb.dlo, fb.dhi);
    cand[t] = q;
    kc[t] = (uint8_t)fb.K;
    s_count(lc, SC_FINAL_BANDED);
    if (early) S.mark |= ST_COUNTED_FINAL;
  }
  tr[t] = S;
  if (dd) dead[t] |= dd;
  });
}

struct AlignOutDev {
  int32_t *score_fwd, *score_rev, *score_prelim, *score_final;
  uint8_t* forward;
  uint32_t *slice_begin, *slice_len, *ref_pos, *ops_len;
};
__global__ void s_align_finish_kernel(SParams p, const STrace* __restrict__ tr, const int32_t* __restrict__ top_full, uint32_t* __restrict__ dead,
                                      AlignOutDev o, unsigned long long* __restrict__ cnt) {
  with_counters(cnt, [&](unsigned long long* lc) {
  const uint32_t t = blockIdx.x * blockDim.x + threadIdx.x;
  if (t >= p.nt) return;
  if (dead[t]) return;
  const STrace S = tr[t];
  if (!s_final_certified(o.score_final[t], top_full[t], p.ge, S.bw, o.ops_len[t])) {
    dead[t] |= SD_FINAL_CHECK;
    s_count(lc, SC_FINAL_REPEATED);
    return;
  }
  o.score_fwd[t] = S.sc[0];
  o.score_rev[t] = S.sc[1];
  o.forward[t] = S.fwd;
  if (o.score_prelim) o.score_prelim[t] = S.sstar;
  o.slice_begin[t] = S.trim.ri;
  o.slice_len[t] = S.trim.len;
  o.ref_pos[t] = S.trim.pos;
  });
}

struct Frac2 { double a, b; };
template <class T>
__global__ void s_scatter_kernel(const uint32_t* __restrict__ list, uint32_t n, const T* __restrict__ src, T* __restrict__ dst) {
  const uint32_t i = blockIdx.x * blockDim.x + threadIdx.x;
  if (i < n && dst) dst[list[i]] = src[i];
}
template <class T>
int scatter(hipStream_t st, const uint32_t* d_list, uint32_t n, const T* src, T* dst) {
  if (!dst || n == 0) return TRACYHIP_OK;
  hipLaunchKernelGGL(s_scatter_kernel<T>, dim3((n + 255) / 256), dim3(256), 0, st, d_list, n, src, dst);
  HIP_TRY(hipGetLastError());
  return TRACYHIP_OK;
}

struct SweepClass { int K; uint32_t lo, hi; };

struct StreamCommon {
  SGeom* geom;
  VoteDesc* vd;
  RowMaxDesc *rm_rest, *rm_trim, *rm_full;
  B16TableDesc* td;
  uint32_t* votes;
  int32_t *ub, *ub1, *top_trim, *top_full;
  int32_t* sc2;
  PairDesc *full, *pre, *fpairs0, *fpairs1, *fpairs2, *cand;
  FrontDesc* fd;
  FrontOut *fo0, *fo1, *fo2;
  int32_t *fs0, *fs1, *fs2;
  uint32_t *fe0, *fe1, *fe2;
  STrace* tr;
  RowEndDesc* re;
  uint32_t* ce;
  uint32_t* dead;
  uint8_t* kc;
  uint32_t* idx;
  ScanPart* part;
  uint32_t* count;
  uint32_t* flist;
  uint32_t* fcount;
  unsigned long long* cnt;
  unsigned long long* bstat;
  uint32_t* ends;
  uint32_t large_stages = 0;
  void layout(Arena& a, uint32_t nt, uint32_t nunits, bool exact, bool want_full_top) {
    geom = a.take<SGeom>(nt);
    vd = a.take<VoteDesc>(nt);
    rm_rest = a.take<RowMaxDesc>(nt);
    rm_trim = a.take<RowMaxDesc>(nt);
    rm_full = want_full_top ? a.take<RowMaxDesc>(nt) : nullptr;
    td = a.take<B16TableDesc>(nt);
    votes = a.take<uint32_t>(2 * (size_t)nt);
    ub = a.take<int32_t>(nt);
    ub1 = a.take<int32_t>(nt);
    top_trim = a.take<int32_t>(nt);
    top_full = want_full_top ? a.take<int32_t>(nt) : nullptr;
    sc2 = a.take<int32_t>(2 * (size_t)nt);
    full = a.take<PairDesc>(2 * (size_t)nt);
    pre = a.take<PairDesc>(std::max<size_t>((exact ? 1 : 2) * (size_t)nt, nunits));
    fpairs0 = a.take<PairDesc>(nunits);
    fpairs1 = a.take<PairDesc>(nunits);
    fpairs2 = a.take<PairDesc>(nunits);
    cand = a.take<PairDesc>(nunits);
    fd = a.take<FrontDesc>(nunits);
    fo0 = a.take<FrontOut>(nunits);
    fo1 = a.take<FrontOut>(nunits);
    fo2 = a.take<FrontOut>(nunits);
    fs0 = a.take<int32_t>(nunits);
    fs1 = a.take<int32_t>(nunits);
    fs2 = a.take<int32_t>(nunits);
    fe0 = a.take<uint32_t>(2 * (size_t)nunits);
    fe1 = a.take<uint32_t>(2 * (size_t)nunits);
    fe2 = a.take<uint32_t>(2 * (size_t)nunits);
    tr = a.take<STrace>(nt);
    re = a.take<RowEndDesc>(nt);
    ce = a.take<uint32_t>(nt);
    dead = a.take<uint32_t>(nt);
    kc = a.take<uint8_t>(nunits);
    idx = a.take<uint32_t>(4 * (size_t)nunits);
    part = a.take<ScanPart>((nunits + kScanBlock - 1) / kScanBlock + 1);
    count = a.take<uint32_t>(4 * 8);
    flist = a.take<uint32_t>(nunits);
    fcount = a.take<uint32_t>(4);
    cnt = a.take<unsigned long long>(SC_COUNT);
    bstat = a.take<unsigned long long>(SB_COUNT * 8);
    ends = a.take<uint32_t>(2 * (size_t)nunits);
  }
};

struct StreamHost {
  std::vector<uint32_t> mf, mt, tl, rn, ridx;
  uint32_t nt = 0;
  std::vector<SweepClass> classes;
  uint64_t lr_tot = 0, tab_tot = 0;
  uint32_t maxmt = 0, maxmf = 0, max_rest = 0;
  uint64_t max_mn = 0;
};

void sweep_order(StreamHost& h, std::vector<uint32_t>& order, const std::vector<int>& kof, bool similar) {
  const uint32_t nt = h.nt;
  h.classes.clear();
  order.clear();
  if (similar) {
    if (nt) h.classes.push_back(SweepClass{kof[0], 0u, nt});
    return;
  }
  order.resize(nt);
  for (uint32_t t = 0; t < nt; ++t) order[t] = t;
  auto before = [&](uint32_t x, uint32_t y) {
    if (kof[x] != kof[y]) return kof[x] > kof[y];
    return (uint64_t)h.mt[x] * h.rn[x] > (uint64_t)h.mt[y] * h.rn[y];
  };
  if (!std::is_sorted(order.begin(), order.end(), before)) std::stable_sort(order.begin(), order.end(), before);
  for (uint32_t i = 0; i < nt;) {
    uint32_t e = i;
    while (e < nt && kof[order[e]] == kof[order[i]]) ++e;
    h.classes.push_back(SweepClass{kof[order[i]], i, e});
    i = e;
  }
}

bool stream_options_ok(const CtxKnobs& k) {
  return !k.no_stream && !k.no_narrow && !k.no_band && !k.no_band16 && !k.no_front && !k.no_prefix && !k.no_vote && !k.no_origin &&
         !k.no_subwindow && !k.no_prelim_origin && !k.no_cq && k.band_w < 0;
}

int workspace_budget(tracyhip_ctx* ctx, uint64_t held, uint64_t* out, bool* from_cache = nullptr) {
  if (from_cache) *from_cache = false;
  if (ctx->ws_limit) { *out = ctx->ws_limit; return TRACYHIP_OK; }
  if (ctx->ws_cache_budget && ctx->ws_cache_held == held && ctx->ws_cache_share == ctx->mem_share) {
    *out = ctx->ws_cache_budget;
    if (from_cache) *from_cache = true;
    return TRACYHIP_OK;
  }
  TRY(workspace_limit(ctx, held, out));
  ctx->ws_cache_budget = *out; ctx->ws_cache_held = held; ctx->ws_cache_share = ctx->mem_share;
  return TRACYHIP_OK;
}
template <class Plan>
int with_fresh_budget(tracyhip_ctx* ctx, Plan plan) {
  bool from_cache = false;
  int rc = plan(&from_cache);
  if (rc == TRACYHIP_ERR_OOM && from_cache) {
    (void)hipGetLastError();
    ctx->ws_cache_budget = 0;
    rc = plan(&from_cache);
  }
  return rc;
}

DpArgs sweep_args(tracyhip_ctx* ctx, const tracyhip_params& p, const void* d_a1, const void* d_a2, int32_t* d_scores, int32_t* d_lastrow) {
  DpArgs a = scoring_args(ctx, &p);
  a.a1 = d_a1; a.a2 = d_a2; a.scores = d_scores;
  a.ckpt = d_lastrow;
  a.lastrow = d_lastrow;
  a.ckpt_B = 0x7fffffffu;
  a.ckpt_narrow = 1;
  return a;
}

bool front_tier_fits(int KB, int32_t halfw, uint32_t max_rest) {
  const uint64_t code_cap = (max_rest + 2u * (uint32_t)halfw + 16u) & ~3u;
  return 4ull * code_cap + b16_table_bytes(KB) + 32ull * kB16RowCap <= 64u * 1024u;
}
bool front_tiers_fit(uint32_t max_rest) { return front_tier_fits(8, 60, max_rest) && front_tier_fits(kFrontK, kFrontHalfW, max_rest); }

int front_tier(tracyhip_ctx* ctx, const tracyhip_params& p, const FrontDesc* fd, uint32_t n, const int16_t* d_qp, const uint8_t* d_codes, const uint32_t* d_row,
               int KB, int32_t halfw, uint32_t max_rest, PairDesc* pairs, FrontOut* fo, int32_t* fs, uint32_t* fe, const FrontOut* prev,
               const uint32_t* list, const uint32_t* list_count) {
  hipStream_t st = ctx->stream;
  Band16Args a{};
  a.pairs = pairs; a.npairs = n; a.index = list; a.count = list_count; a.qp = d_qp; a.codes = d_codes; a.scores = fs; a.ends = fe;
  a.err = static_cast<int32_t*>(ctx->dev[DB_ERR].p); a.go = p.go; a.ge = p.ge; a.hfree = 1; a.row = d_row;
  a.code_cap = (max_rest + 2u * (uint32_t)halfw + 16u) & ~3u;
  if (KB == 0) {
    if (b16_cont_quad_lds(a.code_cap) > 64u * 1024u) return kStreamNo;
  } else if (!front_tier_fits(KB, halfw, max_rest)) return set_error(TRACYHIP_ERR_ARG, "pruned-sweep tier without LDS room (front_tiers_fit not consulted)");
  HIP_TRY(launch_front_place(fd, n, d_row, p.go + p.ge, halfw, pairs, fo, st, prev, list, list_count));
  if (KB == 0) HIP_TRY(launch_band16_cont_quad(a, st));
  else HIP_TRY(launch_band16_cont(KB, a, st, !ctx->knobs.no_cont16));
  HIP_TRY(launch_front_certify(fd, n, d_row, p.go, p.ge, halfw, fs, fe, fo, st, prev, list, list_count));
  return TRACYHIP_OK;
}

__device__ __forceinline__ void s_list_append(bool take, uint32_t i, uint32_t* __restrict__ list, uint32_t* __restrict__ count) {
  __shared__ uint32_t wave_n[4], base;
  const uint32_t wv = threadIdx.x >> 6, L = threadIdx.x & 63u;
  const unsigned long long bal = __ballot(take);
  if (L == 0) wave_n[wv] = (uint32_t)__popcll(bal);
  __syncthreads();
  if (threadIdx.x == 0) {
    const uint32_t tot = wave_n[0] + wave_n[1] + wave_n[2] + wave_n[3];
    base = tot ? atomicAdd(count, tot) : 0u;
  }
  __syncthreads();
  if (!take) return;
  uint32_t at = base + (uint32_t)__popcll(bal & ((1ull << L) - 1ull));
  for (uint32_t k = 0; k < wv; ++k) at += wave_n[k];
  list[at] = i;
}
__global__ __launch_bounds__(256) void s_front_list_kernel(uint32_t n, const FrontOut* __restrict__ prev, uint32_t* __restrict__ list, uint32_t* __restrict__ count,
                                                           FrontOut* __restrict__ next) {
  const uint32_t i = blockIdx.x * 256u + threadIdx.x;
  const bool take = i < n && !prev[i].ok;
  if (i < n && !take) next[i].ok = 0u;
  s_list_append(take, i, list, count);
}
__global__ __launch_bounds__(256) void s_pair_list_kernel(uint32_t n, const PairDesc* __restrict__ pairs, uint32_t* __restrict__ list, uint32_t* __restrict__ count) {
  const uint32_t i = blockIdx.x * 256u + threadIdx.x;
  s_list_append(i < n && !(pairs[i].flags & PAIR_SKIP), i, list, count);
}
hipError_t front_list(tracyhip_ctx* ctx, uint32_t n, const FrontOut* prev, uint32_t* list, uint32_t* count, FrontOut* next) {
  hipLaunchKernelGGL(s_front_list_kernel, dim3((n + 255) / 256), dim3(256), 0, ctx->stream, n, prev, list, count, next);
  return hipGetLastError();
}

__global__ void s_front_fold_kernel(uint32_t n, const FrontOut* __restrict__ fo0, const int32_t* __restrict__ fs0, const uint32_t* __restrict__ fe0,
                                    FrontOut* __restrict__ fo1, int32_t* __restrict__ fs1, uint32_t* __restrict__ fe1) {
  const uint32_t i = blockIdx.x * blockDim.x + threadIdx.x;
  if (i >= n || !fo0[i].ok) return;
  fo1[i] = fo0[i];
  fs1[i] = fs0[i];
  fe1[2 * i] = fe0[2 * i];
  fe1[2 * i + 1] = fe0[2 * i + 1];
}
int front_tiers_run_wide(tracyhip_ctx* ctx, const tracyhip_params& p, StreamCommon& sc, uint32_t n, const int16_t* d_qp, const uint8_t* d_codes,
                         const uint32_t* d_row, uint32_t max_rest, bool after_quads) {
  const bool lists = !ctx->knobs.no_front_lists && n >= ctx->knobs.front_list_min;
  if (lists) HIP_TRY(hipMemsetAsync(sc.fcount, 0, 2 * sizeof(uint32_t), ctx->stream));
  const bool list1 = lists && after_quads;
  if (list1) HIP_TRY(front_list(ctx, n, sc.fo0, sc.flist, sc.fcount, sc.fo1));
  int rc = front_tier(ctx, p, sc.fd, n, d_qp, d_codes, d_row, 8, 60, max_rest, sc.fpairs1, sc.fo1, sc.fs1, sc.fe1, after_quads ? sc.fo0 : nullptr,
                      list1 ? sc.flist : nullptr, list1 ? sc.fcount : nullptr);
  if (rc) return rc;
  if (after_quads) {
    hipLaunchKernelGGL(s_front_fold_kernel, dim3((n + 255) / 256), dim3(256), 0, ctx->stream, n, sc.fo0, sc.fs0, sc.fe0, sc.fo1, sc.fs1, sc.fe1);
    HIP_TRY(hipGetLastError());
  }
  if (lists) HIP_TRY(front_list(ctx, n, sc.fo1, sc.flist, sc.fcount + 1, sc.fo2));
  return front_tier(ctx, p, sc.fd, n, d_qp, d_codes, d_row, kFrontK, kFrontHalfW, max_rest, sc.fpairs2, sc.fo2, sc.fs2, sc.fe2, sc.fo1,
                    lists ? sc.flist : nullptr, lists ? sc.fcount + 1 : nullptr);
}
constexpr int32_t kQuadHalfW = 5;

int front_tiers_run(tracyhip_ctx* ctx, const tracyhip_params& p, StreamCommon& sc, uint32_t n, const int16_t* d_qp, const uint8_t* d_codes, const uint32_t* d_row,
                    uint32_t max_rest) {
  const bool quads = !ctx->knobs.no_quads && n >= ctx->knobs.quad_tier_min;
  int rc = TRACYHIP_OK;
  if (quads) rc = front_tier(ctx, p, sc.fd, n, d_qp, d_codes, d_row, 0, kQuadHalfW, max_rest, sc.fpairs0, sc.fo0, sc.fs0, sc.fe0, nullptr, nullptr, nullptr);
  if (rc == kStreamNo && quads) return front_tiers_run_wide(ctx, p, sc, n, d_qp, d_codes, d_row, max_rest, false);
  if (rc) return rc;
  return front_tiers_run_wide(ctx, p, sc, n, d_qp, d_codes, d_row, max_rest, quads);
}

struct BandLaunch {
  int kind = 0;
  const int16_t* qp = nullptr;
  const uint8_t* codes = nullptr;
  int32_t* scores = nullptr;
  uint32_t* ends = nullptr;
  uint8_t* ops = nullptr;
  const uint64_t* ops_off = nullptr;
  uint32_t* ops_len = nullptr;
  uint32_t code_cap = 0;
  int hfree = 1;
};
int band_stage(tracyhip_ctx* ctx, const tracyhip_params& p, StreamCommon& sc, uint32_t n, uint32_t unit_mod, int stage_no, const BandLaunch& bl, uint64_t cap_bytes) {
  hipStream_t st = ctx->stream;
  uint32_t* count = sc.count + 4 * stage_no;
  const uint32_t nb = (n + kScanBlock - 1) / kScanBlock;
  const int quads = (!ctx->knobs.no_quads && b16_quad_lds(bl.code_cap) <= 64u * 1024u) ? 1 : 0;
  hipLaunchKernelGGL(s_scan_partial_kernel, dim3(nb), dim3(kScanBlock), 0, st, sc.cand, sc.kc, n, bl.kind, quads, sc.part);
  hipLaunchKernelGGL(s_scan_top_kernel, dim3(1), dim3(kScanTop), 0, st, sc.part, nb, count, sc.bstat + SB_COUNT * stage_no);
  hipLaunchKernelGGL(s_scan_place_kernel, dim3(nb), dim3(kScanBlock), 0, st, sc.cand, sc.kc, n, unit_mod, bl.kind, quads, (unsigned long long)cap_bytes, sc.part, sc.idx, sc.dead,
                     sc.bstat + SB_COUNT * stage_no);
  HIP_TRY(hipGetLastError());
  Band16Args a{};
  a.pairs = sc.cand; a.npairs = n; a.qp = bl.qp; a.codes = bl.codes; a.bits = static_cast<uint8_t*>(ctx->dev[DB_BITS].p); a.scores = bl.scores; a.ends = bl.ends;
  a.err = static_cast<int32_t*>(ctx->dev[DB_ERR].p); a.go = p.go; a.ge = p.ge; a.hfree = bl.hfree;
  a.ops = bl.ops; a.ops_off = bl.ops_off; a.ops_len = bl.ops_len; a.code_cap = bl.code_cap;
  Band16Args ak[4] = {a, a, a, a};
  for (int b = 0; b < 4; ++b) { ak[b].index = sc.idx + (size_t)b * n; ak[b].count = count + b; }
  if (!quads) ak[3].npairs = 0;
  TRY(timing_begin(ctx, bl.kind == 0 ? TRACYHIP_TIMER_TRACE : TRACYHIP_TIMER_ORIGIN, 0, 0));
  bool large = false;
  HIP_TRY(launch_band16_counted(bl.kind, ak[0], ak[1], ak[2], ak[3], st, (ctx->b16_fork_ok && !ctx->knobs.no_fork) ? &ctx->b16_fork : nullptr,
                                ctx->knobs.b16_multi_max, &large));
  if (large) ++sc.large_stages;
  TRY(timing_end(ctx));
  return TRACYHIP_OK;
}

uint64_t band_words_cap(uint64_t rows, uint64_t npairs, uint64_t budget_left) {
  const uint64_t worst = rows * 131 + npairs * 10240;
  return std::max<uint64_t>(std::min(worst, budget_left / 2), 1ull << 20);
}
struct OrientStage {
  const void* d_prof;
  const int16_t* d_qp;
  int32_t* d_lastrow;
  bool exact;
  PairDesc* desc_trim;
  std::function<int()> filler;
  std::function<int()> early_tail;
};
int queue_orientation(tracyhip_ctx* ctx, const tracyhip_params& p, const SParams& sp, const StreamHost& h, StreamCommon& sc, const OrientStage& os) {
  hipStream_t st = ctx->stream;
  const uint32_t nt = h.nt;
  const dim3 g256((nt + 255) / 256), b256(256);
  const float* prof = static_cast<const float*>(os.d_prof);
  hipLaunchKernelGGL(s_expand_kernel, g256, b256, 0, st, sc.geom, nt, sc.vd, sc.rm_rest, sc.rm_trim, sc.rm_full, sc.td);
  HIP_TRY(hipGetLastError());
  const bool prep_fork = ctx->b16_fork_ok && !ctx->knobs.no_fork;
  hipStream_t sp1 = st;
  if (prep_fork) {
    HIP_TRY(hipEventRecord(ctx->b16_fork.forked, st));
    HIP_TRY(hipStreamWaitEvent(ctx->b16_fork.side[1], ctx->b16_fork.forked, 0));
    sp1 = ctx->b16_fork.side[1];
    ctx->stream = sp1;
  }
  {
    int rc = timing_begin(ctx, TRACYHIP_TIMER_MISC, 0, h.tab_tot * 2);
    hipError_t e = hipSuccess;
    if (!rc) {
      e = launch_b16_tables(sc.td, nt, os.d_prof, false, p.match, p.mismatch, sub_limit(&p), kTagShift, const_cast<int16_t*>(os.d_qp),
                            static_cast<int32_t*>(ctx->dev[DB_ERR].p), sp1);
      rc = timing_end(ctx);
    }
    ctx->stream = st;
    hipLaunchKernelGGL(rowmax_rest_kernel, dim3(nt), dim3(64), 0, sp1, sc.rm_rest, prof, (float)p.match, (float)p.mismatch, sc.ub, sc.ub1);
    hipLaunchKernelGGL(rowmax_rest_kernel, dim3(nt), dim3(64), 0, sp1, sc.rm_trim, prof, (float)p.match, (float)p.mismatch, sc.top_trim, (int32_t*)nullptr);
    if (sc.rm_full) hipLaunchKernelGGL(rowmax_rest_kernel, dim3(nt), dim3(64), 0, sp1, sc.rm_full, prof, (float)p.match, (float)p.mismatch, sc.top_full, (int32_t*)nullptr);
    hipLaunchKernelGGL(kmer_vote_kernel, dim3(nt), dim3(64), 0, st, sc.vd, prof, ctx->codes(), sc.votes);
    if (prep_fork) {
      HIP_TRY(hipEventRecord(ctx->b16_fork.joined[1], sp1));
      HIP_TRY(hipStreamWaitEvent(st, ctx->b16_fork.joined[1], 0));
    }
    if (rc) return rc;
    HIP_TRY(e);
  }
  hipLaunchKernelGGL(s_orient_plan_kernel, g256, b256, 0, st, sp, sc.geom, sc.votes, sc.ub, sc.ub1, sc.full, sc.pre, sc.fd, sc.tr, sc.cnt);
  HIP_TRY(hipGetLastError());
  DpArgs a = sweep_args(ctx, p, os.d_prof, ctx->codes(), sc.sc2, os.d_lastrow);
  if (!ctx->knobs.no_compact) a.special_blocks = ctx->special_blocks();
  if (sp.use_votes) { a.votes = sc.votes; a.vote_nt = nt; }
  DpArgs ap = a;
  ap.pairs = sc.pre;
  ap.votes = nullptr;
  const uint32_t npre_all = (os.exact ? 1u : 2u) * nt;
  auto front_tiers = [&]() -> int {
    TRY(timing_begin(ctx, TRACYHIP_TIMER_FRONT, 0, 0));
    const int rc = front_tiers_run(ctx, p, sc, nt, os.d_qp, ctx->codes(), reinterpret_cast<const uint32_t*>(os.d_lastrow), h.max_rest);
    const int rc2 = timing_end(ctx);
    return rc ? rc : rc2;
  };
  if (ctx->b16_fork_ok && !ctx->knobs.no_fork) {
    const B16Fork& fk = ctx->b16_fork;
    HIP_TRY(hipEventRecord(fk.forked, st));
    HIP_TRY(hipStreamWaitEvent(fk.side[0], fk.forked, 0));
    ctx->stream = fk.side[0];
    int rc = TRACYHIP_OK;
    {
      DpArgs af = a, apl = ap;
      launch_diag_periods(ctx, &p, h.classes[0].K, 0u, npre_all, true, af, apl);
      if (launch_gotoh_ckpt_front(h.classes[0].K, af, 0u, apl, npre_all, fk.side[0]) != hipSuccess) rc = set_error(TRACYHIP_ERR_HIP, "prefix launch failed");
    }
    if (!rc) rc = front_tiers();
    if (!rc && os.early_tail) {
      hipLaunchKernelGGL(s_orient_early_kernel, g256, b256, 0, fk.side[0], sp, sc.fo1, sc.fs1, sc.fe1, sc.fo2, sc.fs2, sc.fe2, sc.tr);
      if (hipGetLastError() != hipSuccess) rc = set_error(TRACYHIP_ERR_HIP, "early decision launch failed");
      else rc = os.early_tail();
    }
    ctx->stream = st;
    HIP_TRY(hipEventRecord(fk.joined[0], fk.side[0]));
    if (rc) {
      HIP_TRY(hipStreamWaitEvent(st, fk.joined[0], 0));
      return rc;
    }
    if (ctx->knobs.sweeps_alone) HIP_TRY(hipStreamWaitEvent(st, fk.joined[0], 0));
    auto sweeps = [&]() -> int {
      for (const SweepClass& c : h.classes) {
        DpArgs af = a;
        af.pairs = sc.full + 2 * (size_t)c.lo;
        DpArgs apl = ap;
        launch_diag_periods(ctx, &p, c.K, 2 * (c.hi - c.lo), 0u, true, af, apl);
        TRY(timing_begin(ctx, TRACYHIP_TIMER_SCORE, 0, 0));
        const hipError_t e = launch_gotoh_ckpt_front(c.K, af, 2 * (c.hi - c.lo), apl, 0u, st);
        TRY(timing_end(ctx));
        HIP_TRY(e);
      }
      return os.filler ? os.filler() : TRACYHIP_OK;
    };
    const int src = sweeps();
    HIP_TRY(hipStreamWaitEvent(st, fk.joined[0], 0));
    if (src) return src;
  } else {
    bool pre_done = false;
    for (const SweepClass& c : h.classes) {
      DpArgs af = a;
      af.pairs = sc.full + 2 * (size_t)c.lo;
      DpArgs apl = ap;
      launch_diag_periods(ctx, &p, c.K, 2 * (c.hi - c.lo), pre_done ? 0u : npre_all, true, af, apl);
      TRY(timing_begin(ctx, TRACYHIP_TIMER_SCORE, 0, 0));
      HIP_TRY(launch_gotoh_ckpt_front(c.K, af, 2 * (c.hi - c.lo), apl, pre_done ? 0u : npre_all, st));
      TRY(timing_end(ctx));
      pre_done = true;
    }
    TRY(front_tiers());
  }
  hipLaunchKernelGGL(s_orient_decide_kernel, g256, b256, 0, st, sp, sc.geom, sc.votes, sc.ub, sc.sc2, sc.fo1, sc.fs1, sc.fe1, sc.fo2, sc.fs2, sc.fe2, sc.tr, sc.re,
                     sc.dead, sc.cnt, os.desc_trim);
  hipLaunchKernelGGL(row_m_end_kernel, dim3(nt), dim3(64), 0, st, static_cast<const RowEndDesc*>(sc.re), static_cast<const int32_t*>(os.d_lastrow), p.go + p.ge, sc.ce);
  HIP_TRY(hipGetLastError());
  return TRACYHIP_OK;
}

struct PlanHooks {
  std::function<void(uint32_t lo, uint32_t hi, uint32_t tid)> lengths_slice;
  std::function<int()> between;
  std::function<void(uint32_t lo, uint32_t hi, uint32_t tid)> records_slice;
};
int plan_common(tracyhip_ctx* ctx, const tracyhip_params& p, const tracyhip_seqset& sp, const tracyhip_seqset& sr, const uint32_t* ref_index, uint32_t nt,
                uint32_t trim_l, uint32_t trim_r, StreamHost& h, SGeom* geom, const PlanHooks* hooks = nullptr) {
  h = StreamHost{std::move(h.mf), std::move(h.mt), std::move(h.tl), std::move(h.rn), std::move(h.ridx)};
  h.nt = nt;
  h.mf.resize(nt); h.mt.resize(nt); h.tl.resize(nt); h.rn.resize(nt); h.ridx.resize(nt);
  static thread_local std::vector<int> kof_tls;
  std::vector<int>& kof = kof_tls;
  kof.resize(nt);
  bool odd_shape = false, similar = true;
  uint64_t lr_base[kHostThreads], tab_base[kHostThreads];
  {
    TRACYHIP_HOST_SCOPE(hs1, "plan_common.lengths");
    struct Part { uint64_t max_mn, cmin, cmax, lr, tab; uint32_t maxmt, maxmf, bad; int k0; bool odd, onek; };
    Part part[kHostThreads];
    for (auto& x : part) x = Part{0, ~0ull, 0, 0, 0, 0, 0, ~0u, 0, false, true};
    parallel_for(nt, [&](uint32_t lo, uint32_t hi, uint32_t tid) {
      Part x{0, ~0ull, 0, 0, 0, 0, 0, ~0u, 0, false, true};
      for (uint32_t t = lo; t < hi; ++t) {
        h.ridx[t] = ref_index ? ref_index[t] : t;
        if (h.ridx[t] >= sr.count) { x.bad = std::min(x.bad, t); h.ridx[t] = 0; if (sr.count == 0) continue; }
        h.mf[t] = sp.length[t];
        h.rn[t] = sr.length[h.ridx[t]];
        uint32_t l = trim_l, r = trim_r;
        if ((uint64_t)l + r >= h.mf[t]) { l = 0; r = 0; }
        h.tl[t] = l;
        h.mt[t] = h.mf[t] - (l + r);
        x.max_mn = std::max<uint64_t>(x.max_mn, (uint64_t)h.mf[t] + h.rn[t]);
        x.maxmt = std::max(x.maxmt, h.mt[t]);
        x.maxmf = std::max(x.maxmf, h.mf[t]);
        const int K = choose_k(h.mt[t], MODE_QP);
        kof[t] = K;
        if (t == lo) x.k0 = K;
        x.onek = x.onek && K == x.k0;
        x.odd = x.odd || h.mt[t] == 0 || h.rn[t] == 0 || num_passes(h.mt[t], K) != 1;
        const uint64_t c = (uint64_t)h.mt[t] * h.rn[t];
        x.cmin = std::min(x.cmin, c); x.cmax = std::max(x.cmax, c);
        x.lr += 4ull * ((uint64_t)h.rn[t] + 1);
        x.tab += (uint64_t)kB16Codes * b16_table_stride(h.mf[t]);
      }
      part[tid] = x;
      if (hooks && hooks->lengths_slice && x.bad == ~0u) hooks->lengths_slice(lo, hi, tid);
    });
    for (uint32_t i = 0; i < kHostThreads; ++i) { lr_base[i] = h.lr_tot; tab_base[i] = h.tab_tot; h.lr_tot += part[i].lr; h.tab_tot += part[i].tab; }
    uint32_t bad = ~0u;
    uint64_t cmin = ~0ull, cmax = 0;
    int k0 = 0;
    for (const Part& x : part) {
      h.max_mn = std::max(h.max_mn, x.max_mn); h.maxmt = std::max(h.maxmt, x.maxmt); h.maxmf = std::max(h.maxmf, x.maxmf); bad = std::min(bad, x.bad);
      odd_shape = odd_shape || x.odd;
      if (x.cmax == 0 && x.cmin == ~0ull) continue;
      if (!k0) k0 = x.k0;
      similar = similar && x.onek && x.k0 == k0;
      cmin = std::min(cmin, x.cmin); cmax = std::max(cmax, x.cmax);
    }
    similar = similar && cmax <= cmin + cmin / 4;
    if (bad != ~0u) return set_error(TRACYHIP_ERR_ARG, "ref_index[%u] out of range", bad);
  }
  TRY(check_params(&p, h.max_mn));
  if (!(p.ge < 0 && p.go <= 0 && sub_limit(&p) <= kWideScore)) return kStreamNo;
  if (!narrow_ok(&p, h.maxmt, 16)) return kStreamNo;
  if (odd_shape) return kStreamNo;
  static thread_local std::vector<uint32_t> order_tls;
  std::vector<uint32_t>& order = order_tls;
  { TRACYHIP_HOST_SCOPE(hs3, "plan_common.sweep_order"); sweep_order(h, order, kof, similar); }
  if (hooks && hooks->between) TRY(hooks->between());
  TRACYHIP_HOST_SCOPE(hs4, "plan_common.records_and_offsets");
  uint32_t rest_of[kHostThreads] = {};
  const bool in_trace_order = order.empty();
  parallel_for(nt, [&](uint32_t lo_, uint32_t hi_, uint32_t tid) {
   uint32_t max_rest = 0;
   uint64_t lr = lr_base[tid], tab = tab_base[tid];
   for (uint32_t i = lo_; i < hi_; ++i) {
    const uint32_t t = order.empty() ? i : order[i];
    const SweepClass* cls = nullptr;
    for (const SweepClass& c : h.classes) if (i >= c.lo && i < c.hi) { cls = &c; break; }
    SGeom G{};
    G.prof_off = sp.offset[t];
    G.ref_off = sr.offset[h.ridx[t]];
    G.mf = h.mf[t]; G.mt = h.mt[t]; G.tl = h.tl[t]; G.rn = h.rn[t];
    G.full_a = 2 * cls->lo + (i - cls->lo);
    G.full_b = 2 * cls->lo + (cls->hi - cls->lo) + (i - cls->lo);
    const bool front_ok = s_front_ok(&p, G.mt, G.rn);
    G.flags = front_ok ? SG_FRONT_OK : 0u;
    if (front_ok) max_rest = std::max(max_rest, G.mt - kFrontRows);
    if (in_trace_order) {
      for (int o = 0; o < 2; ++o) { G.lr_off[o] = lr; lr += 2ull * ((uint64_t)G.rn + 1); }
      G.tab_stride = b16_table_stride(G.mf);
      G.tab_off = tab;
      tab += (uint64_t)kB16Codes * G.tab_stride;
    }
    geom[t] = G;
   }
   rest_of[tid] = max_rest;
   if (in_trace_order && hooks && hooks->records_slice) hooks->records_slice(lo_, hi_, tid);
  });
  for (uint32_t x : rest_of) h.max_rest = std::max(h.max_rest, x);
  if (!in_trace_order) {
    parallel_for(nt, [&](uint32_t lo, uint32_t hi, uint32_t tid) {
      uint64_t lr = lr_base[tid], tab = tab_base[tid];
      for (uint32_t t = lo; t < hi; ++t) {
        SGeom& G = geom[t];
        for (int o = 0; o < 2; ++o) { G.lr_off[o] = lr; lr += 2ull * ((uint64_t)G.rn + 1); }
        G.tab_stride = b16_table_stride(G.mf);
        G.tab_off = tab;
        tab += (uint64_t)kB16Codes * G.tab_stride;
      }
      if (hooks && hooks->records_slice) hooks->records_slice(lo, hi, tid);
    });
  }
  if (h.max_rest == 0) return kStreamNo;
  if (!front_tiers_fit(h.max_rest)) return kStreamNo;
  return TRACYHIP_OK;
}

int stream_range_verdict(const tracyhip_params& p, const int32_t* herr, const StreamHost& h) {
  if (herr[0] & 1) return kStreamNo;
  if (herr[1] > sub_limit(&p) || herr[2] || herr[3]) return kStreamNo;
  return TRACYHIP_OK;
}

void stats_from_counters(tracyhip_ctx* ctx, const unsigned long long* c, const unsigned long long* bstat, int nstages, const int* stage_timer,
                         uint32_t large_stages) {
  tracyhip_call_stats& s = ctx->stats;
  s.pruned += (uint32_t)c[SC_PRUNED]; s.pruned_uncertified += (uint32_t)c[SC_PRUNED_UNCERT];
  s.prelim_banded += (uint32_t)c[SC_PRELIM_BANDED]; s.prelim_repeated += (uint32_t)c[SC_PRELIM_REPEATED];
  s.final_banded += (uint32_t)c[SC_FINAL_BANDED]; s.final_repeated += (uint32_t)c[SC_FINAL_REPEATED];
  for (int k = 0; k < 2; ++k) { s.allele_pruned[k] += (uint32_t)c[SC_ALLELE_PRUNED0 + k]; s.allele_uncertified[k] += (uint32_t)c[SC_ALLELE_UNCERT0 + k]; }
  for (int k = 0; k < 3; ++k) { s.allele_banded[k] += (uint32_t)c[SC_ALLELE_BANDED0 + k]; s.allele_repeated[k] += (uint32_t)c[SC_ALLELE_REPEATED0 + k]; }
  s.allele_shared_prefix += (uint32_t)c[SC_ALLELE_SHARED];
  for (int i = 0; i < nstages; ++i)
    for (int b = 0; b < SB_LIST_N; ++b) s.band_list_pairs[stage_timer[i] == TRACYHIP_TIMER_TRACE ? 0 : 1][b] += (uint32_t)bstat[SB_COUNT * i + SB_LIST + b];
  s.band_large_launches += large_stages;
  if (ctx->timing) {
    ctx->acc[TRACYHIP_TIMER_SCORE].cells += c[SC_SWEEP_CELLS];
    ctx->acc[TRACYHIP_TIMER_SCORE].bytes += c[SC_SWEEP_BYTES];
    ctx->acc[TRACYHIP_TIMER_DECOMP].cells += c[SC_DECOMP_CELLS];
    ctx->acc[TRACYHIP_TIMER_DECOMP].bytes += c[SC_DECOMP_BYTES];
    ctx->acc[TRACYHIP_TIMER_FRONT].cells += c[SC_FRONT_CELLS];
    ctx->acc[TRACYHIP_TIMER_FRONT].bytes += c[SC_FRONT_BYTES];
    for (int i = 0; i < nstages; ++i) {
      ctx->acc[stage_timer[i]].cells += bstat[SB_COUNT * i + SB_CELLS];
      ctx->acc[stage_timer[i]].bytes += bstat[SB_COUNT * i + SB_BYTES];
    }
  }
  if (ctx->knobs.verbose)
    for (int i = 0; i < nstages; ++i) {
      const unsigned long long* hst = bstat + SB_COUNT * i + SB_HIST;
      const unsigned long long* lst = bstat + SB_COUNT * i + SB_LIST;
      fprintf(stderr, "tracyhip: band stage %d: pairs by diagonals <=8 %llu <=16 %llu <=24 %llu <=32 %llu <=48 %llu <=64 %llu <=96 %llu more %llu; "
              "by strip height 12: %llu 8: %llu 4: %llu quads: %llu\n", i, hst[0], hst[1], hst[2], hst[3], hst[4], hst[5], hst[6], hst[7], lst[0], lst[1], lst[2], lst[3]);
    }
}


struct DeadReason { uint32_t bit; const char* name; };

struct ReadBack {
  int32_t* herr = nullptr;
  unsigned long long *hcnt = nullptr, *hbst = nullptr;
  uint32_t* hdead = nullptr;
  void* extra = nullptr;
  int carve(tracyhip_ctx* ctx, uint32_t nt, size_t extra_bytes) {
    HIP_TRY(ctx->pin[PB_RES].ensure(kErrBytes + sizeof(unsigned long long) * (SC_COUNT + SB_COUNT * 8) + sizeof(uint32_t) * (size_t)nt + extra_bytes));
    herr = static_cast<int32_t*>(ctx->pin[PB_RES].p);
    hcnt = reinterpret_cast<unsigned long long*>(herr + kErrWords + 4);
    hbst = hcnt + SC_COUNT;
    hdead = reinterpret_cast<uint32_t*>(hbst + SB_COUNT * 8);
    extra = hdead + nt;
    return TRACYHIP_OK;
  }
  int queue_verdict(tracyhip_ctx* ctx, hipStream_t st) {
    HIP_TRY(hipMemcpyAsync(herr, ctx->dev[DB_ERR].p, kErrBytes, hipMemcpyDeviceToHost, st));
    return TRACYHIP_OK;
  }
  int queue_counters(const StreamCommon& sc, uint32_t nt, hipStream_t st) {
    HIP_TRY(hipMemcpyAsync(hcnt, sc.cnt, sizeof(unsigned long long) * SC_COUNT, hipMemcpyDeviceToHost, st));
    HIP_TRY(hipMemcpyAsync(hbst, sc.bstat, sizeof(unsigned long long) * SB_COUNT * 8, hipMemcpyDeviceToHost, st));
    HIP_TRY(hipMemcpyAsync(hdead, sc.dead, sizeof(uint32_t) * (size_t)nt, hipMemcpyDeviceToHost, st));
    return TRACYHIP_OK;
  }
};

template <class Fields, class Out>
void carve_all(Arena& a, uint32_t nt, Out& x) {
  Fields::each(x, x, [&](auto& p, auto&, uint32_t per) { a.take_into(p, (size_t)per * nt); });
}
template <class Fields, class To, class From>
void point_all(To& to, const From& from) {
  Fields::each(to, from, [](auto& t, auto& f, uint32_t) { t = f; });
}
template <class Fields, class Out>
int scatter_all(hipStream_t st, const uint32_t* d_list, uint32_t n, Out& compact, Out& o) {
  int rc = TRACYHIP_OK;
  Fields::each(compact, o, [&](auto* src, auto* dst, uint32_t per) {
    if (rc != TRACYHIP_OK) return;
    if constexpr (std::is_same_v<decltype(src), double*>)
      rc = scatter(st, d_list, n, reinterpret_cast<const Frac2*>(src), reinterpret_cast<Frac2*>(dst));
    else
      rc = scatter(st, d_list, n, src, dst);
  });
  return rc;
}
int copy_to_host(hipStream_t st, void* user, const void* dev, size_t bytes) {
  if (user && bytes) HIP_TRY(hipMemcpyAsync(user, dev, bytes, hipMemcpyDeviceToHost, st));
  return TRACYHIP_OK;
}
template <class Fields, class Result, class Out>
int copy_back_all(hipStream_t st, uint32_t nt, const Result& user, Out& o) {
  int rc = TRACYHIP_OK;
  Fields::each(user, o, [&](auto& u, auto& d, uint32_t per) {
    if (rc == TRACYHIP_OK) rc = copy_to_host(st, u, d, sizeof(*d) * per * (size_t)nt);
  });
// ... 901 lines not shown
      TRY(launch_decompose(ctx, a, bpo, maxbc, 0, 0));
      if (build_peaks) { TRY(launch_peaks(ctx, A.bcd, nt, maxbc, d_sig, d_pos, A.peaks)); build_peaks = false; }
      if (peaks_forked) { HIP_TRY(hipStreamWaitEvent(st, ctx->b16_fork.ready[1], 0)); peaks_forked = false; }
      TRY(launch_secdecomp(ctx, A.bcd, nt, maxbc, d_peaks, d_pri, d_sec, d_sd));
      af_pending = ctx->b16_fork_ok && !ctx->knobs.no_fork;
      if (!af_pending) TRY(queue_allelic_fraction());
    }
    hipLaunchKernelGGL(s_status_kernel, g256, b256, 0, st, spm, sc.geom, o.score_trim, A.hst, A.len1, sc.dead, o.status, sc.cnt);
    HIP_TRY(hipGetLastError());

    return TRACYHIP_OK;
  }

  int encode_windows_cq() {
    if (cq_ref_done) return TRACYHIP_OK;
    cq_ref_done = true;
    d_cq_ref = A.cq_ref + kCodePad;
    HIP_TRY(hipMemsetAsync(A.cq_ref, 5, kCodePad, st));
    HIP_TRY(hipMemsetAsync(A.cq_ref + kCodePad + z.er, 5, kCodePad, st));
    HIP_TRY(hipMemsetAsync(A.cq_special, 0, (z.er >> 8) + 2, st));
    HIP_TRY(hipMemsetAsync(A.cq_flag, 0, sizeof(int32_t) * 4, st));
    if (z.er) hipLaunchKernelGGL(encode_cq_kernel, dim3((unsigned)((z.er + 4095) / 4096)), dim3(256), 0, st, d_ref, d_cq_ref, z.er, A.cq_flag, A.cq_special);
    HIP_TRY(hipGetLastError());
    return TRACYHIP_OK;
  }

  int queue_allelic_fraction() {
    const bool fork = af_pending;
    af_pending = false;
    if (fork) {
      HIP_TRY(hipStreamWaitEvent(ctx->b16_fork.side[3], ctx->b16_fork.ready[0], 0));
      ctx->stream = ctx->b16_fork.side[3];
    }
    const int rc = launch_allelic_fraction(ctx, A.bcd, nt, maxbc, d_peaks, d_pri, d_sd, TL, TR, o.fractions, 18ull * std::accumulate(h.mf.begin(), h.mf.end(), 0ull), z.bext);
    ctx->stream = st;
    if (fork) {
      HIP_TRY(hipEventRecord(ctx->b16_fork.joined[3], ctx->b16_fork.side[3]));
      af_forked = true;
    }
    return rc;
  }

  int queue_allele_stages() {
    StreamCommon& sc = A.sc;
    d_cq_sd = A.cq_sd + kCodePad;
    HIP_TRY(hipMemcpyAsync(A.seqs2, d_pri, z.bext, hipMemcpyDeviceToDevice, st));
    HIP_TRY(hipMemcpyAsync(A.seqs2 + z.bext, d_sd, z.bext, hipMemcpyDeviceToDevice, st));
    TRY(encode_windows_cq());
    HIP_TRY(hipMemsetAsync(A.cq_sd, 5, kCodePad, st));
    HIP_TRY(hipMemsetAsync(A.cq_sd + kCodePad + z.bext, 5, kCodePad, st));
    if (z.bext) {
      hipLaunchKernelGGL(encode_cq_kernel, dim3((unsigned)((z.bext + 4095) / 4096)), dim3(256), 0, st, static_cast<const uint8_t*>(d_sd), d_cq_sd, z.bext, A.cq_flag, (uint8_t*)nullptr);
      hipLaunchKernelGGL(cq_rows_kernel, dim3((unsigned)((2 * z.bext + 4095) / 4096)), dim3(256), 0, st, static_cast<const uint8_t*>(A.seqs2), 2 * z.bext, A.cq_flag);
    }
    HIP_TRY(hipGetLastError());
    d_aqp = static_cast<const int16_t*>(ctx->dev[DB_B16TAB_ALLELE0].p);
    TRY(timing_begin(ctx, TRACYHIP_TIMER_MISC, 0, atab_tot * 2));
    HIP_TRY(launch_b16_tables(A.atd, 2 * nt, A.seqs2, true, p.match, p.mismatch, sub_limit(&p), kTagShift, const_cast<int16_t*>(d_aqp), static_cast<int32_t*>(ctx->dev[DB_ERR].p), st));
    TRY(timing_end(ctx));
    const bool share = !kn.no_front_lists && 2 * nt >= kn.front_list_min;
    hipLaunchKernelGGL(s_allele_plan0_kernel, g256x2, b256, 0, st, spm, spd, sc.geom, A.geomd, sc.tr, sc.dead, sc.pre, sc.fd, static_cast<const uint8_t*>(A.seqs2),
                       share ? 1 : 0, sc.cnt);
    HIP_TRY(hipGetLastError());
    if (share) {
      HIP_TRY(hipMemsetAsync(sc.fcount + 2, 0, sizeof(uint32_t), st));
      hipLaunchKernelGGL(s_pair_list_kernel, g256x2, b256, 0, st, 2 * nt, sc.pre, sc.flist, sc.fcount + 2);
      HIP_TRY(hipGetLastError());
    }
    {
      DpArgs a = scoring_args(ctx, &p);
      a.pairs = sc.pre;
      if (share) { a.index = sc.flist; a.count = sc.fcount + 2; }
      a.a1 = A.seqs2; a.a2 = d_cq_ref;
      a.special_blocks = kn.no_compact ? nullptr : A.cq_special;
      a.lastrow = d_lastrow;
      if (af_pending) HIP_TRY(hipEventRecord(ctx->b16_fork.ready[0], st));
      TRY(timing_begin(ctx, TRACYHIP_TIMER_SCORE, 0, 0));
      HIP_TRY(launch_gotoh_front_prefix_cq(a, 2 * nt, st));
      TRY(timing_end(ctx));
    }
    if (af_pending) TRY(give_up(queue_allelic_fraction()));
    TRY(timing_begin(ctx, TRACYHIP_TIMER_FRONT, 0, 0));
    {
      int rc = front_tiers_run(ctx, p, sc, 2 * nt, d_aqp, d_cq_ref, reinterpret_cast<const uint32_t*>(d_lastrow), max_arest);
      if (rc) return give_up(rc);
    }
    TRY(timing_end(ctx));
    hipLaunchKernelGGL(s_allele_plan1_kernel, g256x2, b256, 0, st, spm, spd, sc.geom, A.geomd, sc.tr, sc.fo1, sc.fs1, sc.fe1, sc.fo2, sc.fs2, sc.fe2, A.al, sc.dead, sc.cand,
                       sc.kc, sc.cnt);
    HIP_TRY(hipGetLastError());
    BandLaunch b1;
    b1.kind = 1; b1.qp = d_aqp; b1.codes = d_cq_ref; b1.ends = sc.ends; b1.code_cap = ncap; b1.hfree = 1;
    TRY(band_stage(ctx, p, sc, 2 * nt, nt, 1, b1, ~0ull));
    hipLaunchKernelGGL(s_allele_plan2_kernel, g256x2, b256, 0, st, spm, sc.geom, A.geomd, sc.tr, sc.ends, A.al, sc.dead, sc.cand, sc.kc, kn.no_origin_band ? 0 : 1, sc.cnt);
    HIP_TRY(hipGetLastError());
    BandLaunch b2;
    b2.kind = 0; b2.qp = d_aqp; b2.codes = d_cq_ref; b2.scores = A.ascore; b2.ops = d_opsK[0]; b2.ops_off = A.aops_off; b2.ops_len = A.alen; b2.code_cap = ncap; b2.hfree = 1;
    TRY(band_stage(ctx, p, sc, 2 * nt, nt, 2, b2, words_cap));
    hipLaunchKernelGGL(s_allele_check_kernel, g256x2, b256, 0, st, spm, A.al, A.ascore, A.alen, sc.dead, sc.cnt);
    hipLaunchKernelGGL(s_a12_plan_kernel, g256, b256, 0, st, spm, spd, A.geomd, A.ascore, sc.dead, sc.cand, sc.kc, A.bound, sc.cnt);
    HIP_TRY(hipGetLastError());
    BandLaunch b3;
    b3.kind = 0; b3.qp = d_aqp; b3.codes = d_cq_sd; b3.scores = o.score[2]; b3.ops = d_opsK[2]; b3.ops_off = A.ops2_off; b3.ops_len = o.ops_len[2]; b3.code_cap = ncap; b3.hfree = 0;
    TRY(band_stage(ctx, pglobal, sc, nt, nt, 3, b3, words_cap));
    const DecompOutDev& ko = o;
    hipLaunchKernelGGL(s_decompose_finish_kernel, g256, b256, 0, st, spm, sc.tr, A.al, A.ascore, A.alen, A.bound, sc.dead, ko, sc.cnt);
    HIP_TRY(hipGetLastError());

    return TRACYHIP_OK;
  }

  int read_back() {
    if (af_pending) TRY(queue_allelic_fraction());
    if (af_forked) HIP_TRY(hipStreamWaitEvent(st, ctx->b16_fork.joined[3], 0));
    TRY(rb.carve(ctx, nt, sizeof(int32_t) * 4));
    hcq = static_cast<int32_t*>(rb.extra);
    TRY(rb.queue_verdict(ctx, st));
    HIP_TRY(hipMemcpyAsync(hcq, A.cq_flag, sizeof(int32_t) * 4, hipMemcpyDeviceToHost, st));
    TRY(rb.queue_counters(A.sc, nt, st));
    TRY(await_verdict([this](int rc) { return give_up(rc); }));
    if (hcq[0] & 1) return give_up(kStreamNo);
    static const int stage_timer[4] = {TRACYHIP_TIMER_TRACE, TRACYHIP_TIMER_ORIGIN, TRACYHIP_TIMER_TRACE, TRACYHIP_TIMER_TRACE};
    static const DeadReason reasons[] = {{SD_FRONT, "front"}, {SD_STRAND, "strand"}, {SD_LOSER_WON, "loser won"}, {SD_JUNK, "junk"}, {SD_PRELIM_BAND, "prelim band"},
                                         {SD_PRELIM_CHECK, "prelim check"}, {SD_MEM, "mem"}, {SD_ALLELE_FRONT, "allele front"}, {SD_ALLELE_ORIGIN, "allele origin"},
                                         {SD_ALLELE_BAND, "allele band"}, {SD_ALLELE_CHECK, "allele check"}, {SD_A12_BAND, "a12 band"}, {SD_A12_CHECK, "a12 check"},
                                         {SD_SHAPE, "shape"}};
    list_dead("decompose", A.sc, stage_timer, reasons);
    return TRACYHIP_OK;
  }

  int redo_dead_traces() {
    if (dl.empty()) return TRACYHIP_OK;
    const uint32_t nd = (uint32_t)dl.size();
    HIP_TRY(hipMemcpyAsync(A.dead_list, dl.data(), sizeof(uint32_t) * nd, hipMemcpyHostToDevice, st));
    hipLaunchKernelGGL(s_restore_kernel, dim3(nd), dim3(64), 0, st, A.dead_list, A.sc.geom, A.geomd, A.pri_bak, A.sec_bak, d_pri, d_sec);
    HIP_TRY(hipGetLastError());
    HIP_TRY(ctx_sync(ctx));
    std::vector<uint64_t> bcoff(nd), dcpoff(nd), ooff[3];
    std::vector<uint32_t> bclen(nd);
    for (int k = 0; k < 3; ++k) ooff[k].resize(nd);
    for (uint32_t i = 0; i < nd; ++i) {
      const uint32_t t = dl[i];
      bcoff[i] = bc.bc_offset[t]; bclen[i] = bc.bc_len[t];
      dcpoff[i] = out->dcp_offset[t];
      for (int k = 0; k < 3; ++k) ooff[k][i] = out->ops_offset[k][t];
    }
    tracyhip_decompose_job j = *job;
    sub_job(j, d_prof, d_ref);
    j.bc.ntraces = nd;
    j.bc.signal = nullptr; j.bc.signal_offset = nullptr; j.bc.nsamples = nullptr; j.bc.bcpos = nullptr; j.bc.peaks = d_peaks;
    j.bc.primary = d_pri; j.bc.secondary = d_sec; j.bc.bc_offset = bcoff.data(); j.bc.bc_len = bclen.data();
    tracyhip_decompose_result r{};
    point_all<DecompFields>(r, A.f);
    r.dcp_indel = d_di; r.dcp_err = d_de; r.dcp_offset = dcpoff.data();
    r.secdecomp = d_sd;
    for (int k = 0; k < 3; ++k) { r.ops[k] = d_opsK[k]; r.ops_offset[k] = ooff[k].data(); }
    TRY(host_planned([&]() { return decompose_traces_legacy(ctx, &j, prm, TRACYHIP_MEM_DEVICE, &r); }));
    TRY(scatter_all<DecompFields>(st, A.dead_list, nd, A.f, o));
    HIP_TRY(ctx_sync(ctx));
    return TRACYHIP_OK;
  }

  int copy_back() {
    if (!host) return TRACYHIP_OK;
    TRY(copy_to_host(st, bc.primary, d_pri, z.bext)); TRY(copy_to_host(st, bc.secondary, d_sec, z.bext)); TRY(copy_to_host(st, out->secdecomp, d_sd, z.bext));
    TRY(copy_to_host(st, out->dcp_indel, d_di, z.dext * 4)); TRY(copy_to_host(st, out->dcp_err, d_de, z.dext * 4));
    TRY(copy_back_all<DecompFields>(st, nt, *out, o));
// ... 23 lines not shown
```

tracy_amd/csrc/stream_plan.h:

```cpp
#ifndef TRACY_AMD_STREAM_PLAN_H
#define TRACY_AMD_STREAM_PLAN_H

#include "../../include/tracy_hip.h"
#include "band16.h"
#include "front.h"

namespace tracyhip {

enum : uint32_t {
  SD_FRONT = 1u,
  SD_STRAND = 2u,
  SD_LOSER_WON = 4u,
  SD_JUNK = 8u,
  SD_PRELIM_BAND = 16u,
  SD_PRELIM_CHECK = 32u,
  SD_FINAL_BAND = 64u,
  SD_FINAL_CHECK = 128u,
  SD_MEM = 256u,
  SD_ALLELE_FRONT = 512u,
  SD_ALLELE_ORIGIN = 1024u,
  SD_ALLELE_BAND = 2048u,
  SD_ALLELE_CHECK = 4096u,
  SD_A12_BAND = 8192u,
  SD_A12_CHECK = 16384u,
  SD_SHAPE = 32768u,
};

enum : int {
  SC_PRUNED = 0, SC_PRUNED_UNCERT, SC_PRELIM_BANDED, SC_PRELIM_REPEATED, SC_FINAL_BANDED, SC_FINAL_REPEATED,
  SC_ALLELE_PRUNED0, SC_ALLELE_PRUNED1, SC_ALLELE_UNCERT0, SC_ALLELE_UNCERT1,
  SC_ALLELE_BANDED0, SC_ALLELE_BANDED1, SC_ALLELE_BANDED2, SC_ALLELE_REPEATED0, SC_ALLELE_REPEATED1, SC_ALLELE_REPEATED2,
  SC_SWEEP_CELLS, SC_SWEEP_BYTES,
  SC_DECOMP_CELLS, SC_DECOMP_BYTES,
  SC_FRONT_CELLS, SC_FRONT_BYTES,
  SC_ALLELE_SHARED,
  SC_COUNT
};
enum : int { SB_CELLS = 0, SB_BYTES = 1, SB_WORDS = 2, SB_HIST = 4, SB_HIST_N = 8, SB_LIST = 12, SB_LIST_N = 4, SB_COUNT = 16 };
TR_HD int s_width_bucket(int32_t dmin, int32_t dmax) {
  const int32_t w = dmax - dmin + 1;
  return w <= 8 ? 0 : w <= 16 ? 1 : w <= 24 ? 2 : w <= 32 ? 3 : w <= 48 ? 4 : w <= 64 ? 5 : w <= 96 ? 6 : 7;
}

enum : uint32_t { SG_FRONT_OK = 1u };

struct SGeom {
  uint64_t prof_off;
  uint64_t ref_off;
  uint64_t lr_off[2];
  uint64_t tab_off;
  uint64_t ops_off;
  uint32_t mf, mt, tl, rn;
  uint32_t tab_stride;
  uint32_t full_a, full_b;
  uint32_t flags;
};
struct SGeomD {
  uint64_t bc_off;
  uint64_t sig_off;
  uint64_t dcp_off;
  uint64_t opsk_off[3];
  uint64_t atab_off[2];
  uint64_t alr_off[2];
  uint32_t nsamples, sl, soff, atab_stride;
  uint32_t flags[2];
};

struct TrimRec {
  uint32_t ri;
  uint32_t len;
  uint32_t pos;
  uint32_t pad;
};

struct STrace {
  int32_t sc[2];
  int32_t sstar;
  uint32_t ce;
  uint32_t gap;
  uint32_t shift;
  int32_t bw;
  uint8_t g, cls, rc, fwd;
  uint32_t mark;
  TrimRec trim;
};
enum : uint32_t { ST_EARLY = 1u, ST_COUNTED_PRELIM = 2u, ST_COUNTED_FINAL = 4u };
struct SAllele {
  int32_t sstar;
  uint32_t ce;
  int64_t gap;
  uint32_t shift;
  uint32_t pad;
  TrimRec trim;
};

struct SParams {
  int32_t match, mismatch, go, ge;
  uint32_t nt;
  uint32_t exact;
  uint32_t ncap;
  uint32_t trim_left, trim_right;
  uint32_t use_votes;
  uint32_t split_prefix;
};

TR_HD int64_t s_abs64(int32_t x) { return x < 0 ? -(int64_t)x : (int64_t)x; }
TR_HD int64_t s_best(const SParams& p) { const int64_t b = p.match > p.mismatch ? p.match : p.mismatch; return b > 0 ? b : 0; }

TR_HD TrimRec s_trim_finish(uint32_t ri, uint32_t risize, uint32_t n, uint32_t trim_left, uint32_t trim_right, bool forward) {
  if (ri >= trim_left) { ri -= trim_left; risize += trim_left; }
  if ((uint32_t)(ri + risize + trim_right) < n) risize += trim_right;
  TrimRec r;
  r.ri = ri;
  r.len = (ri <= n) ? ((risize < n - ri) ? risize : n - ri) : 0;
  r.pos = 0;
  if (forward) r.pos = ri;
  else {
    const int32_t offset = (int32_t)n - (int32_t)ri - (int32_t)risize;
// ... 130 lines not shown
```

Baseline: 18450.

## Scan front rows early between prefix forms and queue sweeps before front tiers

Adds a front_scan kernel that finds each pair's best last-row column right after the plain-reference prefix form completes, launched between the two prefix kernel forms. The front tiers then reuse that result instead of rescanning. The main-stream sweeps are also issued before the side-stream front tiers, so the two streams overlap more. This adds a scan launch, extra workspace, and reordering of error and join handling across the two streams.

After: 18450. About the same (-0.0%).

```diff
diff --git a/include/tracy_hip.h b/include/tracy_hip.h
--- a/include/tracy_hip.h
+++ b/include/tracy_hip.h
@@ -89,6 +89,7 @@
   uint32_t prefix_diag_launches;
   uint32_t band_list_pairs[2][4];
   uint32_t band_large_launches;
+  uint32_t front_early_placed;
 } tracyhip_call_stats;
 int tracyhip_last_call_stats(tracyhip_ctx* ctx, tracyhip_call_stats* out);
 const char* tracyhip_last_error(void);
diff --git a/tracy_amd/capi.py b/tracy_amd/capi.py
--- a/tracy_amd/capi.py
+++ b/tracy_amd/capi.py
@@ -64,6 +64,10 @@
 
 class CallStatsBands(CallStatsSweeps):
     _fields_ = [("band_list_pairs", (C.c_uint32 * 4) * 2), ("band_large_launches", C.c_uint32)]
+
+
+class CallStatsFront(CallStatsBands):
+    _fields_ = [("front_early_placed", C.c_uint32)]
 
 
 def library_path():
@@ -174,10 +178,10 @@
         return dict(line.split("=", 1) for line in buf.value.decode().splitlines())
 
     def last_call_stats(self):
-        st = CallStatsBands()
+        st = CallStatsFront()
         _check(lib().tracyhip_last_call_stats(self._h, C.byref(st)))
         out = {}
-        for name, ty in CallStats._fields_ + CallStatsVariants._fields_ + CallStatsSweeps._fields_ + CallStatsBands._fields_:
+        for name, ty in CallStats._fields_ + CallStatsVariants._fields_ + CallStatsSweeps._fields_ + CallStatsBands._fields_ + CallStatsFront._fields_:
             v = getattr(st, name)
             if name == "band_list_pairs":
                 out[name] = [list(row) for row in v]
diff --git a/tracy_amd/csrc/band16.hip b/tracy_amd/csrc/band16.hip
--- a/tracy_amd/csrc/band16.hip
+++ b/tracy_amd/csrc/band16.hip
@@ -86,6 +86,11 @@
   if (prev && prev[u].ok) f.flags |= PAIR_SKIP;
   const FrontOut* known = (prev && !(f.flags & PAIR_SKIP) && prev[u].cstar != 0u) ? prev + u : nullptr;
   front_place_body(w, f, row, goe, halfw, pairs + u, fo + u, known);
+}
+__global__ __launch_bounds__(64) void front_scan_kernel(const FrontDesc* __restrict__ desc, const uint32_t* __restrict__ row, int32_t goe,
+                                                        const uint8_t* __restrict__ special_blocks, FrontOut* __restrict__ fo) {
+  DeviceWave16 w;
+  front_scan_body(w, desc[blockIdx.x], row, goe, special_blocks, fo + blockIdx.x);
 }
 __global__ __launch_bounds__(64) void front_certify_kernel(const FrontDesc* __restrict__ desc, const uint32_t* __restrict__ row, int32_t go, int32_t ge,
                                                            int32_t halfw, const int32_t* __restrict__ scores, const uint32_t* __restrict__ ends,
@@ -255,6 +260,12 @@
   return hipGetLastError();
 }
 
+hipError_t launch_front_scan(const FrontDesc* d_desc, uint32_t n, const uint32_t* row, int32_t goe, const uint8_t* special_blocks, FrontOut* d_fo, hipStream_t s) {
+  if (n == 0) return hipSuccess;
+  hipLaunchKernelGGL(front_scan_kernel, dim3(n), dim3(64), 0, s, d_desc, row, goe, special_blocks, d_fo);
+  return hipGetLastError();
+}
+
 hipError_t launch_front_certify(const FrontDesc* d_desc, uint32_t n, const uint32_t* row, int32_t go, int32_t ge, int32_t halfw, const int32_t* d_scores,
                                 const uint32_t* d_ends, FrontOut* d_fo, hipStream_t s, const FrontOut* d_prev, const uint32_t* d_index,
                                 const uint32_t* d_count) {
diff --git a/tracy_amd/csrc/band16_launch.h b/tracy_amd/csrc/band16_launch.h
--- a/tracy_amd/csrc/band16_launch.h
+++ b/tracy_amd/csrc/band16_launch.h
@@ -39,6 +39,7 @@
 struct FrontOut;
 hipError_t launch_front_place(const FrontDesc* d_desc, uint32_t n, const uint32_t* row, int32_t goe, int32_t halfw, PairDesc* d_pairs, FrontOut* d_fo,
                               hipStream_t s, const FrontOut* d_prev = nullptr, const uint32_t* d_index = nullptr, const uint32_t* d_count = nullptr);
+hipError_t launch_front_scan(const FrontDesc* d_desc, uint32_t n, const uint32_t* row, int32_t goe, const uint8_t* special_blocks, FrontOut* d_fo, hipStream_t s);
 hipError_t launch_front_certify(const FrontDesc* d_desc, uint32_t n, const uint32_t* row, int32_t go, int32_t ge, int32_t halfw, const int32_t* d_scores,
                                 const uint32_t* d_ends, FrontOut* d_fo, hipStream_t s, const FrontOut* d_prev = nullptr, const uint32_t* d_index = nullptr,
                                 const uint32_t* d_count = nullptr);
diff --git a/tracy_amd/csrc/capi.hip b/tracy_amd/csrc/capi.hip
--- a/tracy_amd/csrc/capi.hip
+++ b/tracy_amd/csrc/capi.hip
@@ -234,7 +234,7 @@
     {"no_screen", &CtxKnobs::no_screen}, {"no_band", &CtxKnobs::no_band}, {"no_band16", &CtxKnobs::no_band16},
     {"no_front", &CtxKnobs::no_front}, {"no_prefix", &CtxKnobs::no_prefix}, {"no_vote", &CtxKnobs::no_vote},
     {"no_origin", &CtxKnobs::no_origin}, {"no_subwindow", &CtxKnobs::no_subwindow}, {"no_prelim_origin", &CtxKnobs::no_prelim_origin},
-    {"no_cq", &CtxKnobs::no_cq}, {"no_fused_walk", &CtxKnobs::no_fused_walk}, {"no_cont16", &CtxKnobs::no_cont16}, {"no_decomp_wave", &CtxKnobs::no_decomp_wave}, {"no_af_split", &CtxKnobs::no_af_split}, {"no_front_lists", &CtxKnobs::no_front_lists}, {"no_origin_band", &CtxKnobs::no_origin_band}, {"no_quads", &CtxKnobs::no_quads}, {"no_fork", &CtxKnobs::no_fork}, {"no_early_tail", &CtxKnobs::no_early_tail}, {"sweeps_alone", &CtxKnobs::sweeps_alone}, {"no_sweep_diag", &CtxKnobs::no_sweep_diag}, {"verbose", &CtxKnobs::verbose}};
+    {"no_cq", &CtxKnobs::no_cq}, {"no_fused_walk", &CtxKnobs::no_fused_walk}, {"no_cont16", &CtxKnobs::no_cont16}, {"no_decomp_wave", &CtxKnobs::no_decomp_wave}, {"no_af_split", &CtxKnobs::no_af_split}, {"no_front_lists", &CtxKnobs::no_front_lists}, {"no_origin_band", &CtxKnobs::no_origin_band}, {"no_quads", &CtxKnobs::no_quads}, {"no_fork", &CtxKnobs::no_fork}, {"no_early_tail", &CtxKnobs::no_early_tail}, {"no_front_early_scan", &CtxKnobs::no_front_early_scan}, {"no_sweeps_first", &CtxKnobs::no_sweeps_first}, {"sweeps_alone", &CtxKnobs::sweeps_alone}, {"no_sweep_diag", &CtxKnobs::no_sweep_diag}, {"verbose", &CtxKnobs::verbose}};
 bool same_name(const char* a, const char* b) {
   for (; *a && *b; ++a, ++b)
     if (std::tolower((unsigned char)*a) != std::tolower((unsigned char)*b)) return false;
diff --git a/tracy_amd/csrc/capi_internal.h b/tracy_amd/csrc/capi_internal.h
--- a/tracy_amd/csrc/capi_internal.h
+++ b/tracy_amd/csrc/capi_internal.h
@@ -197,6 +197,8 @@
   bool no_quads = false;
   bool no_fork = false;
   bool no_early_tail = false;
+  bool no_front_early_scan = false;
+  bool no_sweeps_first = false;
   bool sweeps_alone = false;
   bool no_sweep_diag = false;
   bool no_origin_band = false;
diff --git a/tracy_amd/csrc/dp_kernels.h b/tracy_amd/csrc/dp_kernels.h
--- a/tracy_amd/csrc/dp_kernels.h
+++ b/tracy_amd/csrc/dp_kernels.h
@@ -608,13 +608,17 @@
 template <int NC>
 TR_HD uint32_t qp16_byte(uint32_t code, uint32_t row, uint32_t lanecol) { return qp16_row_byte<NC>(row) + code * 256u + 2u * lanecol; }
 template <class W>
+TR_HD bool blocks_are_plain(W& w, const uint8_t* special_blocks, uint64_t a2_off, uint32_t n) {
+  if (!special_blocks) return false;
+  if (n == 0) return true;
+  const uint64_t first = a2_off >> 8, last = (a2_off + n - 1) >> 8;
+  uint32_t seen = 0;
+  for (uint64_t b = first + w.lane(); b <= last; b += 64) seen |= special_blocks[b];
+  return w.ballot(seen != 0) == 0;
+}
+template <class W>
 TR_HD bool reference_is_plain(W& w, const DpArgs& a, const PairDesc& d) {
-  if (!a.special_blocks) return false;
-  if (d.n == 0) return true;
-  const uint64_t first = d.a2_off >> 8, last = (d.a2_off + d.n - 1) >> 8;
-  uint32_t seen = 0;
-  for (uint64_t b = first + w.lane(); b <= last; b += 64) seen |= a.special_blocks[b];
-  return w.ballot(seen != 0) == 0;
+  return blocks_are_plain(w, a.special_blocks, d.a2_off, d.n);
 }
 template <int K, int NC>
 TR_HD void qp_fetch6(const char* tab, uint32_t addr, QpStrip<K>& q) {
diff --git a/tracy_amd/csrc/dp_kernels.hip b/tracy_amd/csrc/dp_kernels.hip
--- a/tracy_amd/csrc/dp_kernels.hip
+++ b/tracy_amd/csrc/dp_kernels.hip
@@ -530,43 +530,50 @@
   return v;
 }
 template <int GL, int KP>
-static hipError_t launch_gotoh_ckpt_front_t(int K, const DpArgs& full, uint32_t nfull, const DpArgs& pre, uint32_t npre, hipStream_t s) {
+static hipError_t launch_gotoh_ckpt_front_t(int K, const DpArgs& full, uint32_t nfull, const DpArgs& pre, uint32_t npre, hipStream_t s,
+                                            const std::function<hipError_t()>* between) {
   static_assert(GL * KP == (int)kFrontRows, "the rows above the kept one");
   const dim3 grid(nfull + (npre + 64 / GL - 1) / (64 / GL));
   auto lds = [](int KK, bool compact) {
     const uint32_t pre_b = lds_bytes_prefix(KP, compact), sw = lds_bytes_sweep16(KK, compact);
     return (pre_b > sw ? pre_b : sw) + lds_pad();
   };
+  hipError_t mid = hipSuccess;
+  auto queue_between = [&]() { if (between && mid == hipSuccess && (mid = hipGetLastError()) == hipSuccess) mid = (*between)(); };
+#define TRACY_FRONT_FORMS(KK, DIAG)                                                                                     \
+  do {                                                                                                                  \
+    if (full.special_blocks) {                                                                                          \
+      hipLaunchKernelGGL((gotoh_ckpt_prefix_kernel<KK, GL, true, KP, DIAG>), grid, dim3(64), lds(KK, true), s, full, nfull, pre, npre); \
+      queue_between();                                                                                                  \
+    }                                                                                                                   \
+    if (mid == hipSuccess) hipLaunchKernelGGL((gotoh_ckpt_prefix_kernel<KK, GL, false, KP, DIAG>), grid, dim3(64), lds(KK, false), s, full, nfull, pre, npre); \
+    if (!full.special_blocks) queue_between();                                                                          \
+  } while (0)
 #define TRACY_FRONT_CASE(KK)                                                                                            \
   case KK:                                                                                                              \
     if constexpr (KK == 15 || KK == 16) {                                                                               \
       if (combo_uses_diag<KK>(full, nfull, pre, npre)) {                                                                \
-        if (full.special_blocks)                                                                                        \
-          hipLaunchKernelGGL((gotoh_ckpt_prefix_kernel<KK, GL, true, KP, true>), grid, dim3(64), lds(KK, true), s, full, nfull, pre, npre); \
-        hipLaunchKernelGGL((gotoh_ckpt_prefix_kernel<KK, GL, false, KP, true>), grid, dim3(64), lds(KK, false), s, full, nfull, pre, npre); \
+        TRACY_FRONT_FORMS(KK, true);                                                                                    \
         break;                                                                                                          \
       }                                                                                                                 \
     }                                                                                                                   \
-    if (full.special_blocks) {                                                                                          \
-       \
-       \
-      hipLaunchKernelGGL((gotoh_ckpt_prefix_kernel<KK, GL, true, KP>), grid, dim3(64), lds(KK, true), s, full, nfull, pre, npre); \
-      hipLaunchKernelGGL((gotoh_ckpt_prefix_kernel<KK, GL, false, KP>), grid, dim3(64), lds(KK, false), s, full, nfull, pre, npre); \
-    } else {                                                                                                            \
-      hipLaunchKernelGGL((gotoh_ckpt_prefix_kernel<KK, GL, false, KP>), grid, dim3(64), lds(KK, false), s, full, nfull, pre, npre); \
-    }                                                                                                                   \
+    TRACY_FRONT_FORMS(KK, false);                                                                                       \
     break;
   switch (K) {
     TRACY_FRONT_CASE(4) TRACY_FRONT_CASE(8) TRACY_FRONT_CASE(12) TRACY_FRONT_CASE(15) TRACY_FRONT_CASE(16)
     default: return hipErrorInvalidValue;
   }
 #undef TRACY_FRONT_CASE
-  return hipGetLastError();
-}
-hipError_t launch_gotoh_ckpt_front(int K, const DpArgs& full, uint32_t nfull, const DpArgs& pre, uint32_t npre, hipStream_t s) {
+#undef TRACY_FRONT_FORMS
+  if (mid != hipSuccess) return mid;
+  return hipGetLastError();
+}
+hipError_t launch_gotoh_ckpt_front(int K, const DpArgs& full, uint32_t nfull, const DpArgs& pre, uint32_t npre, hipStream_t s,
+                                   const std::function<hipError_t()>* between) {
+  if (between && nfull) return hipErrorInvalidValue;
   if (nfull + npre == 0) return hipSuccess;
-  if (nfull == 0 && npre >= front_prefix_tall_min()) return launch_gotoh_ckpt_front_t<(int)kFrontRows / 16, 16>(K, full, nfull, pre, npre, s);
-  return launch_gotoh_ckpt_front_t<kFrontPrefixLanes, kFrontPrefixK>(K, full, nfull, pre, npre, s);
+  if (nfull == 0 && npre >= front_prefix_tall_min()) return launch_gotoh_ckpt_front_t<(int)kFrontRows / 16, 16>(K, full, nfull, pre, npre, s, between);
+  return launch_gotoh_ckpt_front_t<kFrontPrefixLanes, kFrontPrefixK>(K, full, nfull, pre, npre, s, between);
 }
 
 hipError_t launch_gotoh_prefix(int K, const DpArgs& a, uint32_t npairs, hipStream_t s) {
diff --git a/tracy_amd/csrc/front.h b/tracy_amd/csrc/front.h
--- a/tracy_amd/csrc/front.h
+++ b/tracy_amd/csrc/front.h
@@ -34,6 +34,47 @@
 }
 
 template <class W>
+TR_HD void front_scan_row(W& w, const FrontDesc& f, const uint32_t* row, int32_t goe, int32_t& vmax, uint32_t& cstar) {
+  const uint32_t L = w.lane();
+  const uint32_t* r = row + f.row_off;
+  int32_t best = INT32_MIN;
+  uint32_t bc = 0;
+  constexpr uint32_t kRounds = 8;
+  for (uint32_t c0 = 1u; c0 <= f.n; c0 += 64u * kRounds) {
+    uint32_t x[kRounds];
+#pragma unroll
+    for (uint32_t u = 0; u < kRounds; ++u) {
+      const uint32_t c = c0 + 64u * u + L;
+      x[u] = r[c <= f.n ? c : f.n];
+    }
+#pragma unroll
+    for (uint32_t u = 0; u < kRounds; ++u) {
+      const uint32_t c = c0 + 64u * u + L;
+      const int32_t v = front_v(x[u], goe);
+      const bool take = c <= f.n && v > best;
+      best = take ? v : best;
+      bc = take ? c : bc;
+    }
+  }
+  vmax = INT32_MIN;
+  cstar = 0;
+  for (uint32_t l = 0; l < 64u; ++l) {
+    const int32_t v = (int32_t)w.bcast((uint32_t)best, l);
+    const uint32_t c = w.bcast(bc, l);
+    if (c != 0 && (v > vmax || (v == vmax && c < cstar))) { vmax = v; cstar = c; }
+  }
+}
+
+template <class W>
+TR_HD void front_scan_body(W& w, const FrontDesc& f, const uint32_t* row, int32_t goe, const uint8_t* special_blocks, FrontOut* fo) {
+  const bool scan = !(f.flags & PAIR_SKIP) && (!special_blocks || blocks_are_plain(w, special_blocks, f.a2_off, f.n));
+  int32_t vmax = 0;
+  uint32_t cstar = 0;
+  if (scan) front_scan_row(w, f, row, goe, vmax, cstar);
+  if (w.lane() == 0) *fo = cstar ? FrontOut{vmax, cstar, 0u, 0u} : FrontOut{0, 0u, 0u, 0u};
+}
+
+template <class W>
 TR_HD void front_place_body(W& w, const FrontDesc& f, const uint32_t* row, int32_t goe, int32_t halfw, PairDesc* pair, FrontOut* fo,
                             const FrontOut* known = nullptr) {
   const uint32_t L = w.lane();
@@ -52,33 +93,7 @@
   if (known) {
     vmax = known->vmax;
     cstar = known->cstar;
-  } else {
-    const uint32_t* r = row + f.row_off;
-    int32_t best = INT32_MIN;
-    uint32_t bc = 0;
-    constexpr uint32_t kRounds = 8;
-    for (uint32_t c0 = 1u; c0 <= f.n; c0 += 64u * kRounds) {
-      uint32_t x[kRounds];
-#pragma unroll
-      for (uint32_t u = 0; u < kRounds; ++u) {
-        const uint32_t c = c0 + 64u * u + L;
-        x[u] = r[c <= f.n ? c : f.n];
-      }
-#pragma unroll
-      for (uint32_t u = 0; u < kRounds; ++u) {
-        const uint32_t c = c0 + 64u * u + L;
-        const int32_t v = front_v(x[u], goe);
-        const bool take = c <= f.n && v > best;
-        best = take ? v : best;
-        bc = take ? c : bc;
-      }
-    }
-    for (uint32_t l = 0; l < 64u; ++l) {
-      const int32_t v = (int32_t)w.bcast((uint32_t)best, l);
-      const uint32_t c = w.bcast(bc, l);
-      if (c != 0 && (v > vmax || (v == vmax && c < cstar))) { vmax = v; cstar = c; }
-    }
-  }
+  } else front_scan_row(w, f, row, goe, vmax, cstar);
   if (L != 0) return;
   const int32_t dlo = (int32_t)cstar - halfw, dhi = (int32_t)cstar + halfw;
   const uint32_t a = dlo > 1 ? (uint32_t)(dlo - 1) : 0u;
diff --git a/tracy_amd/csrc/launch.h b/tracy_amd/csrc/launch.h
--- a/tracy_amd/csrc/launch.h
+++ b/tracy_amd/csrc/launch.h
@@ -2,6 +2,8 @@
 #define TRACY_AMD_LAUNCH_H
 
 #include <hip/hip_runtime.h>
+
+#include <functional>
 
 #include "dp_kernels.h"
 
@@ -32,7 +34,8 @@
 hipError_t launch_gotoh_origin(int K, int table, int codes, const DpArgs& a, uint32_t npairs, hipStream_t s);
 hipError_t launch_gotoh_ckpt_prefix(int K, const DpArgs& full, uint32_t nfull, const DpArgs& pre, uint32_t npre, hipStream_t s);
 hipError_t launch_gotoh_prefix(int K, const DpArgs& a, uint32_t npairs, hipStream_t s);
-hipError_t launch_gotoh_ckpt_front(int K, const DpArgs& full, uint32_t nfull, const DpArgs& pre, uint32_t npre, hipStream_t s);
+hipError_t launch_gotoh_ckpt_front(int K, const DpArgs& full, uint32_t nfull, const DpArgs& pre, uint32_t npre, hipStream_t s,
+                                   const std::function<hipError_t()>* between = nullptr);
 hipError_t launch_needle(int mode, int K, bool trace, const DpArgs& a, uint32_t npairs, hipStream_t s);
 hipError_t launch_gotoh_walk(const WalkArgs& a, hipStream_t s);
 hipError_t launch_needle_walk(const WalkArgs& a, const uint32_t* bits32, hipStream_t s);
diff --git a/tracy_amd/csrc/stream.hip b/tracy_amd/csrc/stream.hip
--- a/tracy_amd/csrc/stream.hip
+++ b/tracy_amd/csrc/stream.hip
@@ -165,7 +165,8 @@
                                        const int32_t* __restrict__ sc2, const FrontOut* __restrict__ fo1, const int32_t* __restrict__ fs1,
                                        const uint32_t* __restrict__ fe1, const FrontOut* __restrict__ fo2, const int32_t* __restrict__ fs2,
                                        const uint32_t* __restrict__ fe2, STrace* __restrict__ tr, RowEndDesc* __restrict__ re,
-                                       uint32_t* __restrict__ dead, unsigned long long* __restrict__ cnt, PairDesc* __restrict__ desc_trim) {
+                                       uint32_t* __restrict__ dead, unsigned long long* __restrict__ cnt, PairDesc* __restrict__ desc_trim,
+                                       const FrontOut* __restrict__ fscan) {
   with_counters(cnt, [&](unsigned long long* lc) {
   const uint32_t t = blockIdx.x * blockDim.x + threadIdx.x;
   if (t >= p.nt) return;
@@ -182,6 +183,7 @@
   };
   if (S.cls == 0u) {
     s_count(lc, SC_PRUNED);
+    if (fscan && fscan[t].cstar != 0u) s_count(lc, SC_FRONT_EARLY_PLACED);
     fce = s_front_result(t, fo1, fs1, fe1, fo2, fs2, fe2, &s_g);
     if (fce == 0u) { dd |= SD_FRONT; s_count(lc, SC_PRUNED_UNCERT); }
     else if (p.exact) s_o = sc2[o * nt + t];
@@ -476,6 +478,7 @@
   PairDesc *full, *pre, *fpairs0, *fpairs1, *fpairs2, *cand;
   FrontDesc* fd;
   FrontOut *fo0, *fo1, *fo2;
+  FrontOut* fscan;
   int32_t *fs0, *fs1, *fs2;
   uint32_t *fe0, *fe1, *fe2;
   STrace* tr;
@@ -515,6 +518,7 @@
     fo0 = a.take<FrontOut>(nunits);
     fo1 = a.take<FrontOut>(nunits);
     fo2 = a.take<FrontOut>(nunits);
+    fscan = a.take<FrontOut>(nt);
     fs0 = a.take<int32_t>(nunits);
     fs1 = a.take<int32_t>(nunits);
     fs2 = a.take<int32_t>(nunits);
@@ -674,12 +678,12 @@
   fe1[2 * i + 1] = fe0[2 * i + 1];
 }
 int front_tiers_run_wide(tracyhip_ctx* ctx, const tracyhip_params& p, StreamCommon& sc, uint32_t n, const int16_t* d_qp, const uint8_t* d_codes,
-                         const uint32_t* d_row, uint32_t max_rest, bool after_quads) {
+                         const uint32_t* d_row, uint32_t max_rest, bool after_quads, const FrontOut* first_prev) {
   const bool lists = !ctx->knobs.no_front_lists && n >= ctx->knobs.front_list_min;
   if (lists) HIP_TRY(hipMemsetAsync(sc.fcount, 0, 2 * sizeof(uint32_t), ctx->stream));
   const bool list1 = lists && after_quads;
   if (list1) HIP_TRY(front_list(ctx, n, sc.fo0, sc.flist, sc.fcount, sc.fo1));
-  int rc = front_tier(ctx, p, sc.fd, n, d_qp, d_codes, d_row, 8, 60, max_rest, sc.fpairs1, sc.fo1, sc.fs1, sc.fe1, after_quads ? sc.fo0 : nullptr,
+  int rc = front_tier(ctx, p, sc.fd, n, d_qp, d_codes, d_row, 8, 60, max_rest, sc.fpairs1, sc.fo1, sc.fs1, sc.fe1, after_quads ? sc.fo0 : first_prev,
                       list1 ? sc.flist : nullptr, list1 ? sc.fcount : nullptr);
   if (rc) return rc;
   if (after_quads) {
@@ -693,13 +697,13 @@
 constexpr int32_t kQuadHalfW = 5;
 
 int front_tiers_run(tracyhip_ctx* ctx, const tracyhip_params& p, StreamCommon& sc, uint32_t n, const int16_t* d_qp, const uint8_t* d_codes, const uint32_t* d_row,
-                    uint32_t max_rest) {
+                    uint32_t max_rest, const FrontOut* first_prev) {
   const bool quads = !ctx->knobs.no_quads && n >= ctx->knobs.quad_tier_min;
   int rc = TRACYHIP_OK;
-  if (quads) rc = front_tier(ctx, p, sc.fd, n, d_qp, d_codes, d_row, 0, kQuadHalfW, max_rest, sc.fpairs0, sc.fo0, sc.fs0, sc.fe0, nullptr, nullptr, nullptr);
-  if (rc == kStreamNo && quads) return front_tiers_run_wide(ctx, p, sc, n, d_qp, d_codes, d_row, max_rest, false);
+  if (quads) rc = front_tier(ctx, p, sc.fd, n, d_qp, d_codes, d_row, 0, kQuadHalfW, max_rest, sc.fpairs0, sc.fo0, sc.fs0, sc.fe0, first_prev, nullptr, nullptr);
+  if (rc == kStreamNo && quads) return front_tiers_run_wide(ctx, p, sc, n, d_qp, d_codes, d_row, max_rest, false, first_prev);
   if (rc) return rc;
-  return front_tiers_run_wide(ctx, p, sc, n, d_qp, d_codes, d_row, max_rest, quads);
+  return front_tiers_run_wide(ctx, p, sc, n, d_qp, d_codes, d_row, max_rest, quads, first_prev);
 }
 
 struct BandLaunch {
@@ -797,9 +801,11 @@
   ap.pairs = sc.pre;
   ap.votes = nullptr;
   const uint32_t npre_all = (os.exact ? 1u : 2u) * nt;
+  const uint32_t* d_row = reinterpret_cast<const uint32_t*>(os.d_lastrow);
+  const FrontOut* first_prev = nullptr;
   auto front_tiers = [&]() -> int {
     TRY(timing_begin(ctx, TRACYHIP_TIMER_FRONT, 0, 0));
-    const int rc = front_tiers_run(ctx, p, sc, nt, os.d_qp, ctx->codes(), reinterpret_cast<const uint32_t*>(os.d_lastrow), h.max_rest);
+    const int rc = front_tiers_run(ctx, p, sc, nt, os.d_qp, ctx->codes(), d_row, h.max_rest, first_prev);
     const int rc2 = timing_end(ctx);
     return rc ? rc : rc2;
   };
@@ -812,21 +818,14 @@
     {
       DpArgs af = a, apl = ap;
       launch_diag_periods(ctx, &p, h.classes[0].K, 0u, npre_all, true, af, apl);
-      if (launch_gotoh_ckpt_front(h.classes[0].K, af, 0u, apl, npre_all, fk.side[0]) != hipSuccess) rc = set_error(TRACYHIP_ERR_HIP, "prefix launch failed");
-    }
-    if (!rc) rc = front_tiers();
-    if (!rc && os.early_tail) {
-      hipLaunchKernelGGL(s_orient_early_kernel, g256, b256, 0, fk.side[0], sp, sc.fo1, sc.fs1, sc.fe1, sc.fo2, sc.fs2, sc.fe2, sc.tr);
-      if (hipGetLastError() != hipSuccess) rc = set_error(TRACYHIP_ERR_HIP, "early decision launch failed");
-      else rc = os.early_tail();
-    }
-    ctx->stream = st;
-    HIP_TRY(hipEventRecord(fk.joined[0], fk.side[0]));
-    if (rc) {
-      HIP_TRY(hipStreamWaitEvent(st, fk.joined[0], 0));
-      return rc;
-    }
-    if (ctx->knobs.sweeps_alone) HIP_TRY(hipStreamWaitEvent(st, fk.joined[0], 0));
+      const std::function<hipError_t()> scan = [&]() {
+        return launch_front_scan(sc.fd, nt, d_row, p.go + p.ge, apl.special_blocks, sc.fscan, fk.side[0]);
+      };
+      const bool early_scan = !ctx->knobs.no_front_early_scan;
+      if (launch_gotoh_ckpt_front(h.classes[0].K, af, 0u, apl, npre_all, fk.side[0], early_scan ? &scan : nullptr) != hipSuccess)
+        rc = set_error(TRACYHIP_ERR_HIP, "prefix launch failed");
+      else if (early_scan) first_prev = sc.fscan;
+    }
     auto sweeps = [&]() -> int {
       for (const SweepClass& c : h.classes) {
         DpArgs af = a;
@@ -840,7 +839,27 @@
       }
       return os.filler ? os.filler() : TRACYHIP_OK;
     };
-    const int src = sweeps();
+    const bool sweeps_first = !ctx->knobs.no_sweeps_first && !ctx->knobs.sweeps_alone;
+    int src = TRACYHIP_OK;
+    if (!rc && sweeps_first) {
+      ctx->stream = st;
+      src = sweeps();
+      ctx->stream = fk.side[0];
+    }
+    if (!rc && !src) rc = front_tiers();
+    if (!rc && !src && os.early_tail) {
+      hipLaunchKernelGGL(s_orient_early_kernel, g256, b256, 0, fk.side[0], sp, sc.fo1, sc.fs1, sc.fe1, sc.fo2, sc.fs2, sc.fe2, sc.tr);
+      if (hipGetLastError() != hipSuccess) rc = set_error(TRACYHIP_ERR_HIP, "early decision launch failed");
+      else rc = os.early_tail();
+    }
+    ctx->stream = st;
+    HIP_TRY(hipEventRecord(fk.joined[0], fk.side[0]));
+    if (rc || src) {
+      HIP_TRY(hipStreamWaitEvent(st, fk.joined[0], 0));
+      return rc ? rc : src;
+    }
+    if (ctx->knobs.sweeps_alone) HIP_TRY(hipStreamWaitEvent(st, fk.joined[0], 0));
+    if (!sweeps_first) src = sweeps();
     HIP_TRY(hipStreamWaitEvent(st, fk.joined[0], 0));
     if (src) return src;
   } else {
@@ -858,7 +877,7 @@
     TRY(front_tiers());
   }
   hipLaunchKernelGGL(s_orient_decide_kernel, g256, b256, 0, st, sp, sc.geom, sc.votes, sc.ub, sc.sc2, sc.fo1, sc.fs1, sc.fe1, sc.fo2, sc.fs2, sc.fe2, sc.tr, sc.re,
-                     sc.dead, sc.cnt, os.desc_trim);
+                     sc.dead, sc.cnt, os.desc_trim, first_prev);
   hipLaunchKernelGGL(row_m_end_kernel, dim3(nt), dim3(64), 0, st, static_cast<const RowEndDesc*>(sc.re), static_cast<const int32_t*>(os.d_lastrow), p.go + p.ge, sc.ce);
   HIP_TRY(hipGetLastError());
   return TRACYHIP_OK;
@@ -998,6 +1017,7 @@
   for (int k = 0; k < 2; ++k) { s.allele_pruned[k] += (uint32_t)c[SC_ALLELE_PRUNED0 + k]; s.allele_uncertified[k] += (uint32_t)c[SC_ALLELE_UNCERT0 + k]; }
   for (int k = 0; k < 3; ++k) { s.allele_banded[k] += (uint32_t)c[SC_ALLELE_BANDED0 + k]; s.allele_repeated[k] += (uint32_t)c[SC_ALLELE_REPEATED0 + k]; }
   s.allele_shared_prefix += (uint32_t)c[SC_ALLELE_SHARED];
+  s.front_early_placed += (uint32_t)c[SC_FRONT_EARLY_PLACED];
   for (int i = 0; i < nstages; ++i)
     for (int b = 0; b < SB_LIST_N; ++b) s.band_list_pairs[stage_timer[i] == TRACYHIP_TIMER_TRACE ? 0 : 1][b] += (uint32_t)bstat[SB_COUNT * i + SB_LIST + b];
   s.band_large_launches += large_stages;
@@ -2065,7 +2085,7 @@
     if (af_pending) TRY(give_up(queue_allelic_fraction()));
     TRY(timing_begin(ctx, TRACYHIP_TIMER_FRONT, 0, 0));
     {
-      int rc = front_tiers_run(ctx, p, sc, 2 * nt, d_aqp, d_cq_ref, reinterpret_cast<const uint32_t*>(d_lastrow), max_arest);
+      int rc = front_tiers_run(ctx, p, sc, 2 * nt, d_aqp, d_cq_ref, reinterpret_cast<const uint32_t*>(d_lastrow), max_arest, nullptr);
       if (rc) return give_up(rc);
     }
     TRY(timing_end(ctx));
diff --git a/tracy_amd/csrc/stream_plan.h b/tracy_amd/csrc/stream_plan.h
--- a/tracy_amd/csrc/stream_plan.h
+++ b/tracy_amd/csrc/stream_plan.h
@@ -34,6 +34,7 @@
   SC_DECOMP_CELLS, SC_DECOMP_BYTES,
   SC_FRONT_CELLS, SC_FRONT_BYTES,
   SC_ALLELE_SHARED,
+  SC_FRONT_EARLY_PLACED,
   SC_COUNT
 };
 enum : int { SB_CELLS = 0, SB_BYTES = 1, SB_WORDS = 2, SB_HIST = 4, SB_HIST_N = 8, SB_LIST = 12, SB_LIST_N = 4, SB_COUNT = 16 };
```
